# TJUMMG/OCPG

Measured on AMD Instinct MI355X. Metric: clips/sec fwd+bwd (5x384x640, R101), higher is better.
Workload: dtype bf16

## Files before the change

include/ocpg_hip.h:

```cpp
#ifndef OCPG_HIP_H
#define OCPG_HIP_H
#include <stdint.h>

#ifdef __cplusplus
extern "C" {
#endif

int ocpg_msda_fwd_f32(const float* value, const int64_t* shapes, const int64_t* level_start,
                      const float* loc, const float* attn,
                      int N, int S, int M, int D, int L, int Lq, int P,
                      float* out, const int64_t* shapes_host, void* stream);
int ocpg_msda_fwd_f64(const double* value, const int64_t* shapes, const int64_t* level_start,
                      const double* loc, const double* attn,
                      int N, int S, int M, int D, int L, int Lq, int P,
                      double* out, void* stream);

int ocpg_msda_bwd_f32(const float* value, const int64_t* shapes, const int64_t* level_start,
                      const float* loc, const float* attn, const float* grad_out,
                      int N, int S, int M, int D, int L, int Lq, int P,
                      float* grad_value, float* grad_loc, float* grad_attn,
                      const int64_t* shapes_host, void* stream);
int ocpg_msda_bwd_value_f32(const float* loc, const float* attn, const float* grad_out,
                            int N, int S, int M, int D, int L, int Lq, int P,
                            float* grad_value, const int64_t* shapes_host, void* stream);
int ocpg_msda_bwd_locattn_f32(const float* value, const int64_t* shapes, const int64_t* level_start,
                              const float* loc, const float* attn, const float* grad_out,
                              int N, int S, int M, int D, int L, int Lq, int P,
                              float* grad_loc, float* grad_attn, void* stream);
int ocpg_msda_fused_fwd_f32(const float* value, const int64_t* shapes, const int64_t* level_start,
                            const float* qproj, const float* ref,
                            int N, int S, int M, int D, int L, int Lq, int P,
                            float* out, float* loc_out, float* attn_out, void* stream);
int ocpg_msda_fused_bwd_qproj_f32(const float* value, const int64_t* shapes, const int64_t* level_start,
                                  const float* loc, const float* attn, const float* grad_out,
                                  int N, int S, int M, int D, int L, int Lq, int P,
                                  float* grad_qproj, void* stream);
int ocpg_msda_bwd_value_sel_f32(const float* loc, const float* attn, const float* grad_out,
                                int N, int S, int M, int D, int L, int Lq, int P,
                                float* grad_value, const int64_t* shapes_host, int* sel_state, void* stream);
int ocpg_msda_bwd_f64(const double* value, const int64_t* shapes, const int64_t* level_start,
                      const double* loc, const double* attn, const double* grad_out,
                      int N, int S, int M, int D, int L, int Lq, int P,
                      double* grad_value, double* grad_loc, double* grad_attn, void* stream);

int ocpg_msda_sf_fwd_f32(const float* src, const float* wv, const float* bv, const unsigned char* pad,
                         const int64_t* shapes, const int64_t* level_start, const float* loc, const float* attn,
                         int N, int S, int M, int D, int L, int Lq, int P,
                         float* out, float* s, float* beta, void* stream);
int ocpg_msda_sf_bwd_f32(const float* src, const float* wv, const float* bv, const unsigned char* pad,
                         const int64_t* shapes, const int64_t* level_start, const float* loc, const float* attn,
                         const float* grad_out, int N, int S, int M, int D, int L, int Lq, int P,
                         float* grad_src, float* grad_loc, float* grad_attn, void* stream);
int ocpg_msda_sf_bwd_params_f32(const float* grad_out, const float* s, const float* beta, int N, int M, int D, int Lq,
                                float* grad_wv, float* grad_bv, void* stream);

int ocpg_msda_fwd_h16(const void* value, const int64_t* shapes, const int64_t* level_start,
                      const float* loc, const float* attn,
                      int N, int S, int M, int D, int L, int Lq, int P,
                      void* out, const int64_t* shapes_host, int dtype, void* stream);
int ocpg_msda_bwd_h16(const void* value, const int64_t* shapes, const int64_t* level_start,
                      const float* loc, const float* attn, const void* grad_out,
                      int N, int S, int M, int D, int L, int Lq, int P,
                      float* grad_value, float* grad_loc, float* grad_attn,
                      const int64_t* shapes_host, int* sel_state, int dtype, void* stream);
int ocpg_msda_bwd_value_h16(const float* loc, const float* attn, const void* grad_out,
                            int N, int S, int M, int D, int L, int Lq, int P,
                            float* grad_value, const int64_t* shapes_host, int* sel_state, int dtype, void* stream);
int ocpg_msda_bwd_locattn_h16(const void* value, const int64_t* shapes, const int64_t* level_start,
                              const float* loc, const float* attn, const void* grad_out,
                              int N, int S, int M, int D, int L, int Lq, int P,
                              float* grad_loc, float* grad_attn, int dtype, void* stream);
int ocpg_msda_fused_fwd_h16(const void* value, const int64_t* shapes, const int64_t* level_start,
                            const float* qproj, const float* ref,
                            int N, int S, int M, int D, int L, int Lq, int P,
                            void* out, float* loc_out, float* attn_out, int dtype, void* stream);
int ocpg_msda_fused_bwd_qproj_h16(const void* value, const int64_t* shapes, const int64_t* level_start,
                                  const float* loc, const float* attn, const void* grad_out,
                                  int N, int S, int M, int D, int L, int Lq, int P,
                                  float* grad_qproj, int dtype, void* stream);

int ocpg_bn_act_fwd(const void* x, const float* scale, const float* shift, const void* skip, void* y,
                    long long n_outer, int C, long long inner, int relu, int dtype, void* stream);
int ocpg_bn_act_bwd(const void* gy, const void* y, const float* scale, void* gx, void* gskip,
                    long long n_outer, int C, long long inner, int relu, int dtype, void* stream);

int ocpg_gemm_dgrad_bn_tile(long long M, int N, int K);
int ocpg_gemm_dgrad_bn(const void* a, const void* w, const void* c, const void* mask, const float* scale, void* out, void* out_skip,
                       long long M, int N, int K, int dtype, int tile, void* stream);

int ocpg_win_attn_fwd(const void* qkv, const float* biasT, const int* region, float scale, int BW, int NW, int N, int H,
                      int head_dim, void* out, float* lse, int dtype, void* stream);
int ocpg_win_attn_bwd(const void* qkv, const float* bias, const float* biasT, const int* region, float scale, int BW, int NW,
                      int N, int H, int head_dim, const void* out, const void* dout, const float* lse, void* dqkv, float* Dbuf,
                      float* dbiasT, int dtype, void* stream);

int ocpg_win_attn_bwd_mfma(const void* qkv, const float* bias, const float* biasT, const int* region, float scale, int BW, int NW, int N,
                           int H, int head_dim, const void* out, const void* dout, const float* lse, void* dqkv, float* Dbuf, void* dS,
                           int dtype, void* stream);

int ocpg_win_attn_dtable_supported(int N, int head_dim, int dtype, int T);
int ocpg_win_attn_bwd_mfma_dtable(const void* qkv, const float* bias, const float* biasT, const int* region, float scale, int BW, int NW,
                                  int N, int H, int head_dim, const void* out, const void* dout, const float* lse, void* dqkv, float* Dbuf,
                                  const int* tok_code, int code_off, int T, float* partials, float* dtable, int dtype, void* stream);

int ocpg_dynmask_fwd_f32(const float* feats, const float* params, const float* refpix, int BT, int Q, int C, int H, int W,
                         int stride, float* out, float* pre1, void* stream);

int ocpg_dynmask_bwd_pre_f32(const float* dout, const float* pre1, const float* params, int BT, int Q, int C, int H, int W,
                             int stride, float* dpre, float* part, float* w0d, void* stream);
int ocpg_dynmask_bwd_fin_f32(const float* part, const float* params, const float* refpix, const float* dw0, int BT, int Q, int C,
                             int H, int W, float* dparams, float* dref, void* stream);

int ocpg_im2col3x3_nhwc(const void* x, int N, int H, int W, int C, int stride, int dil, void* cols, int dtype, void* stream);
int ocpg_col2im3x3_nhwc(const void* dcols, int N, int H, int W, int C, int stride, int dil, void* dx, int dtype, void* stream);

int ocpg_conv3x3_mfma_fwd(const void* x, const void* w, const float* scale, const float* bias, int relu, int N, int H, int W,
                          int Cin, int Cout, int stride, void* y, void* stream);
int ocpg_conv3x3_mfma_fwd_cols(const void* x, const void* w, const float* scale, const float* bias, int relu, int N, int H, int W, int Cin,
                               int Cout, int stride, void* y, void* cols, void* stream);
int ocpg_conv3x3_mfma_dgrad(const void* dy, const void* wT, int N, int H, int W, int Cin, int Cout, int stride, void* dx,
                            void* stream);
int ocpg_conv3x3_mfma_dgrad_masked(const void* dy, const void* wT, const void* mask_y, const float* scale, int N, int H, int W, int Cin,
                                   int Cout, int stride, void* dx, void* stream);
int ocpg_conv3x3_mfma_dgrad_w(const void* dy, const void* w, const void* mask_y, const float* scale, int N, int H, int W, int Cin, int Cout,
                              int stride, void* dx, void* stream);
int ocpg_conv3x3_mfma_body_splits(long long M, int ncols, int kchannels);
int ocpg_conv3x3_mfma_fwd_bn_splitk(const void* x, const void* w, const float* scale, const float* shift, int relu, int N, int H, int W, int Cin,
                                    int Cout, int stride, int splits, float* part, void* y, void* stream);
int ocpg_conv3x3_mfma_dgrad_w_splitk(const void* dy, const void* w, const void* mask_y, const float* scale, int N, int H, int W, int Cin,
                                     int Cout, int stride, int splits, float* part, void* dx, void* stream);
int ocpg_conv3x3_mfma_wgrad_splits(int N, int H, int W, int Cin, int Cout, int stride);
int ocpg_conv3x3_mfma_wgrad(const void* gz, const void* x, int N, int H, int W, int Cin, int Cout, int stride, void* part, void* stream);
int ocpg_conv3x3_mfma_fwd_cols_h16(const void* x, const void* w, const float* scale, const float* bias, int relu, int N, int H, int W, int Cin,
                                   int Cout, int stride, void* y, void* cols, int dtype, void* stream);
int ocpg_conv3x3_mfma_dgrad_w_h16(const void* dy, const void* w, const void* mask_y, const float* scale, int N, int H, int W, int Cin, int Cout,
                                  int stride, void* dx, int dtype, void* stream);
int ocpg_conv3x3_mfma_wgrad_h16(const void* gz, const void* x, int N, int H, int W, int Cin, int Cout, int stride, void* part, int dtype,
                                void* stream);
int ocpg_conv3x3_mfma_dgrad_w_s2(const void* dy, const void* w, const void* mask_y, const float* scale, int N, int H, int W, int Cin, int Cout,
                                 int stride, void* dx, void* stream);
int ocpg_conv3x3_mfma_dgrad_w_s2_h16(const void* dy, const void* w, const void* mask_y, const float* scale, int N, int H, int W, int Cin, int Cout,
                                     int stride, void* dx, int dtype, void* stream);

int ocpg_conv3x3_mfma_splits(int N, int H, int W, int Cin, int Cout, int stride);
int ocpg_conv3x3_mfma_fwd_splitk(const void* x, const void* w, const float* bias, int N, int H, int W, int Cin, int Cout, int stride,
                                 int splits, float* part, void* y, int out_dt, void* cols, void* stream);
int ocpg_conv3x3_mfma_fwd_splitk_h16(const void* x, const void* w, const float* bias, int N, int H, int W, int Cin, int Cout, int stride,
                                     int splits, float* part, void* y, int out_dt, void* cols, int dtype, void* stream);

int ocpg_gemm(const void* A, const void* B, void* C, const void* bias, int dtype, int out_dtype, int transA, int transB,
              long long M, long long N, long long K, long long lda, long long ldb, long long ldc, long long batch,
              long long strideA, long long strideB, long long strideC, float alpha, float beta, void* stream);
long long ocpg_gemm_plans(void);
long long ocpg_gemm_tuned(long long* changed);
long long ocpg_gemm_tune_rejected(void);
void ocpg_gemm_set_tuning(int on);
long long ocpg_gemm_export_picks(long long* buf, long long cap_pairs);
int ocpg_gemm_import_picks(const long long* buf, long long n_pairs);
int ocpg_gemm_bn_act(const void* A, const void* W, void* D, const float* scale, const float* shift, const void* skip, int relu, int dtype,
                     long long M, long long N, long long K, void* stream);

int ocpg_levelset_fwd_f32(const float* x, const float* feats, const float* box, int Lr, int N, int C, int CF, int h, int w, float* sums,
                          float* coef, float* loss, void* stream);
int ocpg_levelset_bwd_f32(const float* x, const float* feats, const float* box, const float* coef, const float* gloss, int Lr, int N,
                          int C, int CF, int h, int w, float* gx, float* gfeat, void* stream);
int ocpg_proj_fwd_f32(const float* x, const float* tcmax, const float* trmax, const float* tcmean, const float* trmean, int Lr, int B,
                      int T, int H, int W, float* colstat, float* rowstat, float* IU, float* loss, void* stream);
int ocpg_proj_bwd_f32(const float* x, const float* tcmax, const float* trmax, const float* tcmean, const float* trmean,
                      const float* colstat, const float* rowstat, const float* IU, const float* gloss, int Lr, int B, int T, int H, int W,
                      float* Gc, float* Gr, float* gx, void* stream);

int ocpg_matcher_cost_f32(const float* logits, const float* boxes, const float* masks, long long sl, long long sb, long long st,
                          long long sq, const float* gt, const float* tboxes, const float* valid, const long long* labels, int Lr,
                          int B, int T, int Q, int K, int h, int w, float wc, float wb, float wg, float wm, float wd, float* sums,
                          float* cost, int* bad, void* stream);

int ocpg_dropout_add_ln_fwd(const void* x, const float* res, const float* gamma, const float* beta, long long R, int C, float eps, float p,
                            unsigned long long seed, unsigned long long offset, const unsigned long long* rng_base, int x_dtype, float* y,
                            float* mean, float* rstd, void* stream);
int ocpg_dropout_add_ln_bwd(const float* gy, const void* x, const float* res, const float* gamma, const float* mean, const float* rstd,
                            long long R, int C, float p, unsigned long long seed, unsigned long long offset, const unsigned long long* rng_base,
                            int x_dtype, void* gx, float* gres, float* dgb_part, void* stream);
long long ocpg_dropout_add_ln_bwd_slots(long long R);
int ocpg_dropout_add_ln_fwd_ex(const void* x, const float* res, const float* gamma, const float* beta, long long R, int C, float eps, float p,
                               unsigned long long seed, unsigned long long offset, const unsigned long long* rng_base, int x_dtype, float* y,
                               float* mean, float* rstd, const float* addend, float* y_add, void* y_lp, int lp_dtype, void* stream);
int ocpg_dropout_add_ln_bwd_ex(const void* g0, int g0_dtype, const void* g1, int g1_dtype, const void* g2, int g2_dtype, const void* x,
                               const float* res, const float* gamma, const float* mean, const float* rstd, long long R, int C, float p,
                               unsigned long long seed, unsigned long long offset, const unsigned long long* rng_base, int x_dtype, void* gx,
                               float* gres, float* dgb_part, float* gxsum_part, void* stream);
int ocpg_bias_relu_dropout_fwd(const void* a, const void* bias, long long R, int C, float p, unsigned long long seed,
                               unsigned long long offset, const unsigned long long* rng_base, int dtype, void* h, void* stream);
int ocpg_bias_relu_dropout_bwd(const void* gh, const void* h, long long R, int C, float p, int dtype, void* ga, float* dbias_part,
                               void* stream);
long long ocpg_bias_relu_dropout_bwd_slots(long long R, int C, int dtype);

int ocpg_multi_cast(const long long* srcs, const long long* dsts, const long long* numels, const long long* chunk_prefix, int n,
                    long long total_chunks, int src_dtype, int dst_dtype, void* stream);
int ocpg_multi_cast_sum(const long long* srcs, const long long* dsts, const long long* numels, const long long* chunk_prefix,
                        const long long* splits, const long long* strides, int n, long long total_chunks, int src_dtype, int dst_dtype,
                        void* stream);
long long ocpg_colsum_blocks(long long R);
int ocpg_colsum_partials(const void* x, long long R, int C, int dtype, float* part, void* stream);

int ocpg_grad_norm_clip(const long long* grads, const long long* numels, const long long* chunk_prefix, int n, long long total_chunks,
                        float max_norm, float* partials, float* norm_and_coef, void* stream);
int ocpg_adamw_step(const long long* params, const long long* grads, const long long* exp_avg, const long long* exp_avg_sq,
                    const long long* numels, const long long* chunk_prefix, const float* lr, const float* weight_decay, int n,
                    long long total_chunks, const float* norm_and_coef, double beta1, double beta2, double eps, long long step, void* stream);
int ocpg_grad_norm_clip_amp(const long long* grads, const long long* numels, const long long* chunk_prefix, int n, long long total_chunks,
                            float max_norm, float* partials, const float* grad_scale, const float* found_inf, double beta1, double beta2,
                            float* amp_state, void* stream);
int ocpg_adamw_step_amp(const long long* params, const long long* grads, const long long* exp_avg, const long long* exp_avg_sq,
                        const long long* numels, const long long* chunk_prefix, const float* lr, const float* weight_decay, int n,
                        long long total_chunks, const float* amp_state, double beta1, double beta2, double eps, void* stream);

int ocpg_det_loss_fwd_f32(const float* logits, const float* boxes, const long long* src, const float* valid, const long long* labels,
                          const float* tboxes, const float* num_boxes, float alpha, int Lr, int B, int T, int Q, int K, float* loss, int* bad,
                          void* stream);
int ocpg_det_loss_bwd_f32(const float* logits, const float* boxes, const long long* src, const float* valid, const long long* labels,
                          const float* tboxes, const float* num_boxes, const float* gloss, float alpha, int Lr, int B, int T, int Q, int K,
                          float* glogits, float* gboxes, void* stream);

int ocpg_spectral_gate_fwd(const void* X, const float* coef, const float* high, int N, int C, int hw, float* out, void* stream);
int ocpg_spectral_c2p(const void* X, const float* coef, const float* high, int N, int C, int hw, void* pair, int dtype, void* stream);
int ocpg_spectral_p2c(const void* pair, const void* Xs, const float* coef, const float* high, int N, int C, int hw, void* out, float* part,
                      int dtype, void* stream);
int ocpg_spectral_gate_bwd(const float* gout, const void* X, const float* coef, const float* high, int N, int C, int hw, void* dX, float* part,
                           void* stream);

int ocpg_masked_ce_fwd_f32(const float* x, const float* w, const float* t, int Lr, long long per_layer, float* part, void* stream);
int ocpg_masked_ce_bwd_f32(const float* x, const float* w, const float* t, const float* gloss, int Lr, long long per_layer, float* gx,
                           void* stream);

int ocpg_attn_smallk_fwd(const void* q, long long ldq, const void* k, long long ldk, const void* v, long long ldv,
                         const unsigned char* key_pad, float scale, int Lq, int B, int H, int hd, int Lk, float pdrop,
                         unsigned long long seed, unsigned long long offset, const unsigned long long* rng_base, void* out,
                         long long ldo, float* lse, int dtype, void* stream);
int ocpg_attn_smallk_bwd(const void* q, long long ldq, const void* k, long long ldk, const void* v, long long ldv,
                         const unsigned char* key_pad, const void* dout, long long ldo, const float* lse, float scale, int Lq,
                         int B, int H, int hd, int Lk, float pdrop, unsigned long long seed, unsigned long long offset,
                         const unsigned long long* rng_base, void* dq, long long lddq, float* dk, float* dv, int dtype, void* stream);

int ocpg_attn_longk_fwd(const void* q, long long ldq, const void* k, long long ldk, const void* v, long long ldv,
                        const unsigned char* key_pad, float scale, int Lq, int B, int H, int hd, int Lk, float pdrop,
                        unsigned long long seed, unsigned long long offset, const unsigned long long* rng_base, void* out,
                        long long ldo, float* lse, int dtype, void* stream);
int ocpg_attn_longk_bwd(const void* q, long long ldq, const void* k, long long ldk, const void* v, long long ldv,
                        const unsigned char* key_pad, const void* dout, long long ldo, const void* out, long long ldout,
                        const float* lse, float scale, int Lq, int B, int H, int hd, int Lk, float pdrop, unsigned long long seed,
                        unsigned long long offset, const unsigned long long* rng_base, void* dq, long long lddq, float* dk, float* dv,
                        int dtype, void* stream);

int ocpg_lfm_dft_supported(int H, int W);
int ocpg_lfm_dft_split(int L);
int ocpg_lfm_spectrum_fwd(const float* x, const float* coef, const float* high, int N, int H, int W, int C, const void* tw_h, const void* tw_w,
                          float norm, void* tmp, void* pair, int pair_dt, void* stream);
int ocpg_lfm_spectrum_inv(const void* pair, int pair_dt, const float* coef, const float* high, const void* z_saved, float* coef_part, int N, int H,
                          int W, int C, const void* tw_h, const void* tw_w, float norm, void* tmp, const float* residual, float* out, void* stream);
int ocpg_window_means3x3_fwd(const float* x, long long planes, int h, int w, int as_bf16, float* out, void* stream);
int ocpg_window_means3x3_bwd(const float* gm, long long planes, int h, int w, float* dx, void* stream);
int ocpg_window_sums3x3_cl_bands(int h);
int ocpg_window_sums3x3_cl(const float* x, int N, int h, int w, int C, int as_bf16, float* part, void* stream);
int ocpg_window_means3x3_bwd_cl(const float* gm, int N, int h, int w, int C, const float* addend, float* dx, void* stream);

int ocpg_mso_conv3x3(const void* in, int in_dt, int relu_in, const void* w, int w_dt, const float* bias, const float* addend, int NA,
                     const void* mask, int mask_dt, const float* residual, void* out, int out_dt, int NB, int H, int W, int C,
                     int co_total, int compute_dt, void* stream);
int ocpg_mso_wgrad_rows(int NB, int H, int C, int compute_dt);
int ocpg_mso_wgrad(const void* x, int x_dt, int relu_in, const float* g, float* part, float* part_bias, int accumulate, int NB, int H, int W,
                   int C, int co, int rows_per_band, int compute_dt, void* stream);
int ocpg_bilinear_nhwc_fwd(const float* in, int NB, int H, int W, int C, int HO, int WO, float* out, void* stream);
int ocpg_bilinear_nhwc_bwd(const float* gout, int NB, int H, int W, int C, int HO, int WO, float* gin, void* stream);

int ocpg_small_linear_fwd(const void* x, int x_f32, const void* w, const void* b, int R, int Cin, int Cout, int relu, void* y, void* stream);
int ocpg_small_linear_bwd(const void* gy, int gy_f32, const void* x, int x_f32, const void* w, const void* y_relu, int R, int Cin, int Cout,
                          void* gx, void* gw, void* gb, void* stream);
int ocpg_small_linear_fwd_h16(const void* x, int x_f32, const void* w, const void* b, int R, int Cin, int Cout, int relu, void* y, int dtype,
                              void* stream);
int ocpg_small_linear_bwd_h16(const void* gy, int gy_f32, const void* x, int x_f32, const void* w, const void* y_relu, int R, int Cin, int Cout,
                              void* gx, void* gw, void* gb, int dtype, void* stream);
int ocpg_small_linear_f32_fwd(const float* x, const float* w, const float* b, int R, int Cin, int Cout, float* y, void* stream);
int ocpg_small_linear_f32_bwd(const float* gy, const float* x, const float* w, int R, int Cin, int Cout, float* gx, float* gw, float* gb, void* stream);

int ocpg_layernorm_blocks(long long rows);
int ocpg_layernorm_fwd(const void* x, int x_f32, const float* gamma, const float* beta, long long rows, int C, float eps, void* y, int y_f32,
                       float* mean, float* rstd, void* stream);
int ocpg_layernorm_bwd(const void* gy, int gy_f32, const void* x, int x_f32, const float* gamma, const float* mean, const float* rstd,
                       long long rows, int C, void* dx, int dx_f32, float* part_g, float* part_b, void* stream);

long long ocpg_groupnorm_cl_work(long long N, int HW, int C, int G);
int ocpg_groupnorm_cl_fwd(const void* x, int x_dtype, const float* gamma, const float* beta, long long N, int HW, int C, int G, float eps,
                          float* y, float* mean, float* rstd, float* work, void* stream);
int ocpg_groupnorm_cl_bwd(const float* gy, const void* x, int x_dtype, const float* gamma, const float* mean, const float* rstd, long long N,
                          int HW, int C, int G, void* dx, float* part, float* work, void* stream);
int ocpg_groupnorm_cl2cl_fwd(const void* x, int x_dtype, const float* gamma, const float* beta, long long N, int HW, int C, int G, float eps,
                             float* y, float* mean, float* rstd, float* work, void* stream);
int ocpg_groupnorm_cl2cl_bwd(const float* gy, const void* x, int x_dtype, const float* gamma, const float* mean, const float* rstd, long long N,
                             int HW, int C, int G, void* dx, float* part, float* work, void* stream);

int ocpg_gather_rows_bwd(const float* g, const long long* order, const long long* seg, int T, int H, float* out, void* stream);
int ocpg_relpos_bias_fwd(const float* table, const long long* idx, int N, long long ldi, int H, float* bias, float* bias_t, void* stream);
int ocpg_relpos_bias_bwd(const float* g, const long long* order, const long long* seg, int T, int H, int N, int transposed, float* out,
                         void* stream);

int ocpg_gather_rows_pad(const void* x, const long long* idx, long long B, long long S, long long M, long long row_bytes, void* out,
                         void* stream);

int ocpg_graph_replace_memsets(void* hip_graph, int* n_replaced);
int ocpg_graph_stats(void* hip_graph, long long* out9);
int ocpg_graph_memcpy_nodes(void* hip_graph, long long* out, int cap);

int ocpg_text_gate_rows(int Lk);
int ocpg_text_gate_splits(int L);
int ocpg_text_gate_fwd_h16(const float* x, const void* Kp, const void* Vp, const float* c, const float* bo, const unsigned char* key_pad,
                           float scale, int B, int L, int C, int H, int Lk, float* out, int dtype, void* stream);
int ocpg_text_gate_bwd_h16(const float* x, const float* g, const void* Kp, const void* Vp, const float* c, const float* bo,
                           const unsigned char* key_pad, float scale, int B, int L, int C, int H, int Lk, float* dx, float* part, void* ws,
                           int dtype, void* stream);

int ocpg_mask_tail_f32(const float* src, int K, int N, int hs, int ws, int up, int crop_h, int crop_w, int out_h, int out_w, int mode,
                       float thr, float bg, int on_value, void* out, void* stream);

int ocpg_jf_counts_u8(const unsigned char* gt, const unsigned char* res, int T, int H, int W, int G, int R, int radius, int void_label,
                      int all_pairs, int* counts, void* stream);

long long ocpg_sim_heat_workspace(int F, int h, int w, int total);
int ocpg_sim_heat_f32(const float* feat, int F, int h, int w, int C, int n_obj, const int* obj_frame, const int* cand_off_host,
                      const int* cand_off, const int* cand_xy, const int* box, float* heat, int* choice, float* score, void* workspace,
                      void* stream);

int ocpg_refmask_counts_f32(const float* src, int B, int Q, int hs, int ws, int up, const int* geom_host, const int* geom,
                            const unsigned char* gt, const long long* gt_off, int max_out_h, int max_out_w, float thr, int invert,
                            int* counts, void* stream);

const char* ocpg_hip_version(void);

#ifdef __cplusplus
}
#endif
#endif
```

ocpg_amd/_lib.py:

```python
import ctypes
import os

import torch

_HERE = os.path.dirname(os.path.abspath(__file__))
LIB_PATH = os.environ.get("OCPG_HIP_LIB") or os.path.join(_HERE, "lib", "libocpg_hip.so")
_lib = None

_i64p = ctypes.c_void_p
_vp = ctypes.c_void_p
_int = ctypes.c_int

SIGNATURES = {
    "ocpg_msda_fwd_f32": [_vp, _i64p, _i64p, _vp, _vp] + [_int] * 7 + [_vp, _vp, _vp],
    "ocpg_msda_fwd_f64": [_vp, _i64p, _i64p, _vp, _vp] + [_int] * 7 + [_vp, _vp],
    "ocpg_msda_bwd_f32": [_vp, _i64p, _i64p, _vp, _vp, _vp] + [_int] * 7 + [_vp, _vp, _vp, _vp, _vp],
    "ocpg_msda_bwd_value_f32": [_vp, _vp, _vp] + [_int] * 7 + [_vp, _vp, _vp],
    "ocpg_msda_fused_fwd_f32": [_vp, _i64p, _i64p, _vp, _vp] + [_int] * 7 + [_vp, _vp, _vp, _vp],
    "ocpg_msda_fused_bwd_qproj_f32": [_vp, _i64p, _i64p, _vp, _vp, _vp] + [_int] * 7 + [_vp, _vp],
    "ocpg_msda_bwd_value_sel_f32": [_vp, _vp, _vp] + [_int] * 7 + [_vp, _vp, _vp, _vp],
    "ocpg_msda_bwd_locattn_f32": [_vp, _i64p, _i64p, _vp, _vp, _vp] + [_int] * 7 + [_vp, _vp, _vp],
    "ocpg_msda_bwd_f64": [_vp, _i64p, _i64p, _vp, _vp, _vp] + [_int] * 7 + [_vp, _vp, _vp, _vp],
    "ocpg_msda_sf_fwd_f32": [_vp, _vp, _vp, _vp, _i64p, _i64p, _vp, _vp] + [_int] * 7 + [_vp, _vp, _vp, _vp],
    "ocpg_msda_sf_bwd_f32": [_vp, _vp, _vp, _vp, _i64p, _i64p, _vp, _vp, _vp] + [_int] * 7 + [_vp, _vp, _vp, _vp],
    "ocpg_msda_sf_bwd_params_f32": [_vp, _vp, _vp] + [_int] * 4 + [_vp, _vp, _vp],
    "ocpg_msda_fwd_h16": [_vp, _i64p, _i64p, _vp, _vp] + [_int] * 7 + [_vp, _vp, _int, _vp],
    "ocpg_msda_bwd_h16": [_vp, _i64p, _i64p, _vp, _vp, _vp] + [_int] * 7 + [_vp, _vp, _vp, _vp, _vp, _int, _vp],
    "ocpg_msda_bwd_value_h16": [_vp, _vp, _vp] + [_int] * 7 + [_vp, _vp, _vp, _int, _vp],
    "ocpg_msda_bwd_locattn_h16": [_vp, _i64p, _i64p, _vp, _vp, _vp] + [_int] * 7 + [_vp, _vp, _int, _vp],
    "ocpg_msda_fused_fwd_h16": [_vp, _i64p, _i64p, _vp, _vp] + [_int] * 7 + [_vp, _vp, _vp, _int, _vp],
    "ocpg_msda_fused_bwd_qproj_h16": [_vp, _i64p, _i64p, _vp, _vp, _vp] + [_int] * 7 + [_vp, _int, _vp],
    "ocpg_bn_act_fwd": [_vp, _vp, _vp, _vp, _vp, ctypes.c_longlong, _int, ctypes.c_longlong, _int, _int, _vp],
    "ocpg_bn_act_bwd": [_vp, _vp, _vp, _vp, _vp, ctypes.c_longlong, _int, ctypes.c_longlong, _int, _int, _vp],
    "ocpg_gemm_dgrad_bn_tile": [ctypes.c_longlong, _int, _int],
    "ocpg_gemm_dgrad_bn": [_vp] * 7 + [ctypes.c_longlong, _int, _int, _int, _int, _vp],
    "ocpg_dynmask_fwd_f32": [_vp, _vp, _vp] + [_int] * 6 + [_vp, _vp, _vp],
    "ocpg_dynmask_bwd_pre_f32": [_vp, _vp, _vp] + [_int] * 6 + [_vp, _vp, _vp, _vp],
    "ocpg_dynmask_bwd_fin_f32": [_vp, _vp, _vp, _vp] + [_int] * 5 + [_vp, _vp, _vp],
    "ocpg_conv3x3_mfma_fwd": [_vp, _vp, _vp, _vp] + [_int] * 7 + [_vp, _vp],
    "ocpg_conv3x3_mfma_fwd_cols": [_vp, _vp, _vp, _vp] + [_int] * 7 + [_vp, _vp, _vp],
    "ocpg_conv3x3_mfma_dgrad": [_vp, _vp] + [_int] * 6 + [_vp, _vp],
    "ocpg_conv3x3_mfma_dgrad_masked": [_vp, _vp, _vp, _vp] + [_int] * 6 + [_vp, _vp],
    "ocpg_conv3x3_mfma_dgrad_w": [_vp, _vp, _vp, _vp] + [_int] * 6 + [_vp, _vp],
    "ocpg_conv3x3_mfma_splits": [_int] * 6,
    "ocpg_conv3x3_mfma_wgrad_splits": [_int] * 6,
    "ocpg_conv3x3_mfma_body_splits": [ctypes.c_longlong, _int, _int],
    "ocpg_conv3x3_mfma_fwd_bn_splitk": [_vp, _vp, _vp, _vp] + [_int] * 8 + [_vp, _vp, _vp],
    "ocpg_conv3x3_mfma_dgrad_w_splitk": [_vp, _vp, _vp, _vp] + [_int] * 7 + [_vp, _vp, _vp],
    "ocpg_conv3x3_mfma_wgrad": [_vp, _vp] + [_int] * 6 + [_vp, _vp],
    "ocpg_conv3x3_mfma_fwd_cols_h16": [_vp, _vp, _vp, _vp] + [_int] * 7 + [_vp, _vp, _int, _vp],
    "ocpg_conv3x3_mfma_dgrad_w_h16": [_vp, _vp, _vp, _vp] + [_int] * 6 + [_vp, _int, _vp],
    "ocpg_conv3x3_mfma_wgrad_h16": [_vp, _vp] + [_int] * 6 + [_vp, _int, _vp],
    "ocpg_conv3x3_mfma_dgrad_w_s2": [_vp, _vp, _vp, _vp] + [_int] * 6 + [_vp, _vp],
    "ocpg_conv3x3_mfma_dgrad_w_s2_h16": [_vp, _vp, _vp, _vp] + [_int] * 6 + [_vp, _int, _vp],
    "ocpg_conv3x3_mfma_fwd_splitk": [_vp, _vp, _vp] + [_int] * 7 + [_vp, _vp, _int, _vp, _vp],
    "ocpg_conv3x3_mfma_fwd_splitk_h16": [_vp, _vp, _vp] + [_int] * 7 + [_vp, _vp, _int, _vp, _int, _vp],
    "ocpg_gemm": [_vp, _vp, _vp, _vp] + [_int] * 4 + [ctypes.c_longlong] * 10 + [ctypes.c_float, ctypes.c_float, _vp],
    "ocpg_gemm_plans": [],
    "ocpg_gemm_tuned": [_vp],
    "ocpg_gemm_tune_rejected": [],
    "ocpg_gemm_set_tuning": [_int],
    "ocpg_gemm_export_picks": [_vp, ctypes.c_longlong],
    "ocpg_gemm_import_picks": [_vp, ctypes.c_longlong],
    "ocpg_window_means3x3_fwd": [_vp, ctypes.c_longlong, _int, _int, _int, _vp, _vp],
    "ocpg_window_means3x3_bwd": [_vp, ctypes.c_longlong, _int, _int, _vp, _vp],
    "ocpg_window_sums3x3_cl_bands": [_int],
    "ocpg_window_sums3x3_cl": [_vp, _int, _int, _int, _int, _int, _vp, _vp],
    "ocpg_window_means3x3_bwd_cl": [_vp, _int, _int, _int, _int, _vp, _vp, _vp],
    "ocpg_mso_conv3x3": [_vp, _int, _int, _vp, _int, _vp, _vp, _int, _vp, _int, _vp, _vp, _int] + [_int] * 6 + [_vp],
    "ocpg_mso_wgrad_rows": [_int] * 4,
    "ocpg_mso_wgrad": [_vp, _int, _int, _vp, _vp, _vp] + [_int] * 8 + [_vp],
    "ocpg_bilinear_nhwc_fwd": [_vp] + [_int] * 6 + [_vp, _vp],
    "ocpg_bilinear_nhwc_bwd": [_vp] + [_int] * 6 + [_vp, _vp],
    "ocpg_small_linear_fwd": [_vp, _int, _vp, _vp, _int, _int, _int, _int, _vp, _vp],
    "ocpg_small_linear_bwd": [_vp, _int, _vp, _int, _vp, _vp, _int, _int, _int, _vp, _vp, _vp, _vp],
    "ocpg_small_linear_fwd_h16": [_vp, _int, _vp, _vp, _int, _int, _int, _int, _vp, _int, _vp],
    "ocpg_small_linear_bwd_h16": [_vp, _int, _vp, _int, _vp, _vp, _int, _int, _int, _vp, _vp, _vp, _int, _vp],
    "ocpg_small_linear_f32_fwd": [_vp, _vp, _vp, _int, _int, _int, _vp, _vp],
    "ocpg_small_linear_f32_bwd": [_vp, _vp, _vp, _int, _int, _int, _vp, _vp, _vp, _vp],
    "ocpg_layernorm_blocks": [ctypes.c_longlong],
    "ocpg_groupnorm_cl_work": [ctypes.c_longlong, _int, _int, _int],
    "ocpg_groupnorm_cl_fwd": [_vp, _int, _vp, _vp, ctypes.c_longlong, _int, _int, _int, ctypes.c_float, _vp, _vp, _vp, _vp, _vp],
    "ocpg_groupnorm_cl_bwd": [_vp, _vp, _int, _vp, _vp, _vp, ctypes.c_longlong, _int, _int, _int, _vp, _vp, _vp, _vp],
    "ocpg_groupnorm_cl2cl_fwd": [_vp, _int, _vp, _vp, ctypes.c_longlong, _int, _int, _int, ctypes.c_float, _vp, _vp, _vp, _vp, _vp],
    "ocpg_groupnorm_cl2cl_bwd": [_vp, _vp, _int, _vp, _vp, _vp, ctypes.c_longlong, _int, _int, _int, _vp, _vp, _vp, _vp],
    "ocpg_layernorm_fwd": [_vp, _int, _vp, _vp, ctypes.c_longlong, _int, ctypes.c_float, _vp, _int, _vp, _vp, _vp],
    "ocpg_layernorm_bwd": [_vp, _int, _vp, _int, _vp, _vp, _vp, ctypes.c_longlong, _int, _vp, _int, _vp, _vp, _vp],
    "ocpg_gather_rows_bwd": [_vp, _vp, _vp, _int, _int, _vp, _vp],
    "ocpg_relpos_bias_fwd": [_vp, _vp, _int, ctypes.c_longlong, _int, _vp, _vp, _vp],
    "ocpg_relpos_bias_bwd": [_vp, _vp, _vp, _int, _int, _int, _int, _vp, _vp],
    "ocpg_gather_rows_pad": [_vp, _vp] + [ctypes.c_longlong] * 4 + [_vp, _vp],
    "ocpg_graph_replace_memsets": [_vp, _vp],
    "ocpg_graph_stats": [_vp, _vp],
    "ocpg_graph_memcpy_nodes": [_vp, _vp, _int],
    "ocpg_gemm_bn_act": [_vp] * 6 + [_int, _int] + [ctypes.c_longlong] * 3 + [_vp],
    "ocpg_levelset_fwd_f32": [_vp] * 3 + [_int] * 6 + [_vp] * 4,
    "ocpg_levelset_bwd_f32": [_vp] * 5 + [_int] * 6 + [_vp] * 3,
    "ocpg_proj_fwd_f32": [_vp] * 5 + [_int] * 5 + [_vp] * 5,
    "ocpg_proj_bwd_f32": [_vp] * 9 + [_int] * 5 + [_vp] * 4,
    "ocpg_matcher_cost_f32": [_vp] * 3 + [ctypes.c_longlong] * 4 + [_vp] * 4 + [_int] * 7 + [ctypes.c_float] * 5 + [_vp] * 4,
    "ocpg_dropout_add_ln_fwd": [_vp] * 4 + [ctypes.c_longlong, _int, ctypes.c_float, ctypes.c_float, ctypes.c_ulonglong, ctypes.c_ulonglong, _vp, _int]
                               + [_vp] * 4,
    "ocpg_dropout_add_ln_bwd": [_vp] * 6 + [ctypes.c_longlong, _int, ctypes.c_float, ctypes.c_ulonglong, ctypes.c_ulonglong, _vp, _int] + [_vp] * 4,
    "ocpg_dropout_add_ln_bwd_slots": [ctypes.c_longlong],
    "ocpg_dropout_add_ln_fwd_ex": [_vp] * 4 + [ctypes.c_longlong, _int, ctypes.c_float, ctypes.c_float, ctypes.c_ulonglong, ctypes.c_ulonglong, _vp, _int]
                                  + [_vp] * 6 + [_int, _vp],
    "ocpg_dropout_add_ln_bwd_ex": [_vp, _int] * 3 + [_vp] * 5 + [ctypes.c_longlong, _int, ctypes.c_float, ctypes.c_ulonglong, ctypes.c_ulonglong, _vp, _int]
                                  + [_vp] * 5,
    "ocpg_bias_relu_dropout_fwd": [_vp, _vp, ctypes.c_longlong, _int, ctypes.c_float, ctypes.c_ulonglong, ctypes.c_ulonglong, _vp, _int, _vp, _vp],
    "ocpg_bias_relu_dropout_bwd": [_vp, _vp, ctypes.c_longlong, _int, ctypes.c_float, _int, _vp, _vp, _vp],
    "ocpg_bias_relu_dropout_bwd_slots": [ctypes.c_longlong, _int, _int],
    "ocpg_multi_cast": [_vp] * 4 + [_int, ctypes.c_longlong, _int, _int, _vp],
    "ocpg_multi_cast_sum": [_vp] * 6 + [_int, ctypes.c_longlong, _int, _int, _vp],
    "ocpg_colsum_blocks": [ctypes.c_longlong],
    "ocpg_grad_norm_clip": [_vp] * 3 + [_int, ctypes.c_longlong, ctypes.c_float, _vp, _vp, _vp],
    "ocpg_adamw_step": [_vp] * 8 + [_int, ctypes.c_longlong, _vp, ctypes.c_double, ctypes.c_double, ctypes.c_double, ctypes.c_longlong, _vp],
    "ocpg_grad_norm_clip_amp": [_vp] * 3 + [_int, ctypes.c_longlong, ctypes.c_float, _vp, _vp, _vp, ctypes.c_double, ctypes.c_double, _vp, _vp],
    "ocpg_adamw_step_amp": [_vp] * 8 + [_int, ctypes.c_longlong, _vp, ctypes.c_double, ctypes.c_double, ctypes.c_double, _vp],
    "ocpg_lfm_dft_supported": [_int, _int],
    "ocpg_lfm_dft_split": [_int],
    "ocpg_lfm_spectrum_fwd": [_vp, _vp, _vp] + [_int] * 4 + [_vp, _vp, ctypes.c_float, _vp, _vp, _int, _vp],
    "ocpg_lfm_spectrum_inv": [_vp, _int, _vp, _vp, _vp, _vp] + [_int] * 4 + [_vp, _vp, ctypes.c_float, _vp, _vp, _vp, _vp],
    "ocpg_colsum_partials": [_vp, ctypes.c_longlong, _int, _int, _vp, _vp],
    "ocpg_det_loss_fwd_f32": [_vp] * 7 + [ctypes.c_float] + [_int] * 5 + [_vp] * 3,
    "ocpg_det_loss_bwd_f32": [_vp] * 8 + [ctypes.c_float] + [_int] * 5 + [_vp] * 3,
    "ocpg_spectral_gate_fwd": [_vp] * 3 + [_int] * 3 + [_vp, _vp],
    "ocpg_spectral_gate_bwd": [_vp] * 4 + [_int] * 3 + [_vp, _vp, _vp],
    "ocpg_spectral_c2p": [_vp] * 3 + [_int] * 3 + [_vp, _int, _vp],
    "ocpg_spectral_p2c": [_vp] * 4 + [_int] * 3 + [_vp, _vp, _int, _vp],
    "ocpg_masked_ce_fwd_f32": [_vp] * 3 + [_int, ctypes.c_longlong, _vp, _vp],
    "ocpg_masked_ce_bwd_f32": [_vp] * 4 + [_int, ctypes.c_longlong, _vp, _vp],
    "ocpg_im2col3x3_nhwc": [_vp] + [_int] * 6 + [_vp, _int, _vp],
    "ocpg_col2im3x3_nhwc": [_vp] + [_int] * 6 + [_vp, _int, _vp],
    "ocpg_attn_smallk_fwd": [_vp, ctypes.c_longlong, _vp, ctypes.c_longlong, _vp, ctypes.c_longlong, _vp, ctypes.c_float] + [_int] * 5
                            + [ctypes.c_float, ctypes.c_ulonglong, ctypes.c_ulonglong, _vp, _vp, ctypes.c_longlong, _vp, _int, _vp],
    "ocpg_attn_smallk_bwd": [_vp, ctypes.c_longlong, _vp, ctypes.c_longlong, _vp, ctypes.c_longlong, _vp, _vp, ctypes.c_longlong, _vp,
                             ctypes.c_float] + [_int] * 5 + [ctypes.c_float, ctypes.c_ulonglong, ctypes.c_ulonglong, _vp, _vp, ctypes.c_longlong,
                                                             _vp, _vp, _int, _vp],
    "ocpg_attn_longk_fwd": [_vp, ctypes.c_longlong, _vp, ctypes.c_longlong, _vp, ctypes.c_longlong, _vp, ctypes.c_float] + [_int] * 5
                           + [ctypes.c_float, ctypes.c_ulonglong, ctypes.c_ulonglong, _vp, _vp, ctypes.c_longlong, _vp, _int, _vp],
    "ocpg_attn_longk_bwd": [_vp, ctypes.c_longlong, _vp, ctypes.c_longlong, _vp, ctypes.c_longlong, _vp, _vp, ctypes.c_longlong, _vp,
                            ctypes.c_longlong, _vp, ctypes.c_float] + [_int] * 5 + [ctypes.c_float, ctypes.c_ulonglong, ctypes.c_ulonglong, _vp,
                                                                                    _vp, ctypes.c_longlong, _vp, _vp, _int, _vp],
    "ocpg_text_gate_rows": [_int],
    "ocpg_text_gate_splits": [_int],
    "ocpg_text_gate_fwd_h16": [_vp] * 6 + [ctypes.c_float] + [_int] * 5 + [_vp, _int, _vp],
    "ocpg_text_gate_bwd_h16": [_vp] * 7 + [ctypes.c_float] + [_int] * 5 + [_vp, _vp, _vp, _int, _vp],
    "ocpg_mask_tail_f32": [_vp] + [_int] * 10 + [ctypes.c_float, ctypes.c_float, _int, _vp, _vp],
    "ocpg_jf_counts_u8": [_vp, _vp] + [_int] * 8 + [_vp, _vp],
    "ocpg_refmask_counts_f32": [_vp] + [_int] * 5 + [_vp] * 4 + [_int, _int, ctypes.c_float, _int, _vp, _vp],
    "ocpg_sim_heat_workspace": [_int] * 4,
    "ocpg_sim_heat_f32": [_vp] + [_int] * 5 + [_vp] * 10,
    "ocpg_win_attn_fwd": [_vp, _vp, _vp, ctypes.c_float] + [_int] * 5 + [_vp, _vp, _int, _vp],
    "ocpg_win_attn_bwd": [_vp, _vp, _vp, _vp, ctypes.c_float] + [_int] * 5 + [_vp] * 6 + [_int, _vp],
    "ocpg_win_attn_bwd_mfma": [_vp, _vp, _vp, _vp, ctypes.c_float] + [_int] * 5 + [_vp] * 6 + [_int, _vp],
    "ocpg_win_attn_dtable_supported": [_int] * 4,
    "ocpg_win_attn_bwd_mfma_dtable": [_vp, _vp, _vp, _vp, ctypes.c_float] + [_int] * 5 + [_vp] * 6 + [_int, _int, _vp, _vp, _int, _vp],
}


_TIMING = {"on": False, "events": []}
_UNTIMED = ("ocpg_sim_heat_workspace", "ocpg_text_gate_rows", "ocpg_text_gate_splits", "ocpg_win_attn_dtable_supported", "ocpg_conv3x3_mfma_body_splits", "ocpg_gemm_dgrad_bn_tile", "ocpg_conv3x3_mfma_wgrad_splits", "ocpg_window_sums3x3_cl_bands", "ocpg_lfm_dft_supported", "ocpg_lfm_dft_split", "ocpg_conv3x3_mfma_splits", "ocpg_gemm_set_tuning", "ocpg_gemm_export_picks", "ocpg_gemm_import_picks", "ocpg_colsum_blocks", "ocpg_mso_wgrad_rows", "ocpg_gemm_plans", "ocpg_gemm_tuned", "ocpg_gemm_tune_rejected", "ocpg_bias_relu_dropout_bwd_slots", "ocpg_dropout_add_ln_bwd_slots", "ocpg_groupnorm_cl_work")


def enable_kernel_timing(on=True):
    _TIMING["on"] = on
    _TIMING["events"] = []


def collect_kernel_timing(work=None):
    torch.cuda.synchronize()
    out = {}
    for name, args, e0, e1 in _TIMING["events"]:
        d = out.setdefault(name, {"ms": 0.0, "n": 0, "work": 0.0, "modelled": 0})
        d["ms"] += e0.elapsed_time(e1)
        d["n"] += 1
        w = work(name, args) if work is not None else None
        if isinstance(w, tuple):
            d["work_lowp"] = d.get("work_lowp", 0.0) + (w[0] if w[1] else 0.0)
            w = w[0]
        if w is not None:
            d["work"] += w
            d["modelled"] += 1
    _TIMING["events"] = []
    _TIMING["on"] = False
    return out


CENSUS = {"on": False, "calls": {}}
CENSUS_ALSO = {"ocpg_conv3x3_mfma_dgrad_w_s2": "ocpg_conv3x3_mfma_dgrad_w", "ocpg_conv3x3_mfma_dgrad_w_s2_h16": "ocpg_conv3x3_mfma_dgrad_w_h16",
               "ocpg_dropout_add_ln_fwd_ex": "ocpg_dropout_add_ln_fwd", "ocpg_dropout_add_ln_bwd_ex": "ocpg_dropout_add_ln_bwd"}


def census(on=True):
    CENSUS["on"] = on
    if on:
        CENSUS["calls"] = {}
    return CENSUS["calls"]


class _Lib:

    def __init__(self, cdll):
        self._cdll = cdll

    def __getattr__(self, name):
        fn = getattr(self._cdll, name)
        if name not in SIGNATURES or name in _UNTIMED:
            setattr(self, name, fn)
            return fn
        timed = not name.startswith("ocpg_msda_")

        def call(*a):
            if CENSUS["on"]:
                rc = fn(*a)
                if rc == 0:
                    for k in (name, CENSUS_ALSO.get(name)):
                        if k is not None:
                            CENSUS["calls"][k] = CENSUS["calls"].get(k, 0) + 1
                return rc
            if not (timed and _TIMING["on"]):
                return fn(*a)
            e0, e1 = torch.cuda.Event(enable_timing=True), torch.cuda.Event(enable_timing=True)
            e0.record()
            rc = fn(*a)
            e1.record()
            _TIMING["events"].append((name, tuple(getattr(x, "value", x) for x in a), e0, e1))
            return rc
        setattr(self, name, call)
        return call


def lib():
    global _lib
    if _lib is None:
        if not os.path.exists(LIB_PATH):
            raise RuntimeError(
                f"{LIB_PATH} not found: build it with `python -m ocpg_amd.csrc.build` "
                "(hipcc --offload-arch=gfx950). The HIP extension is mandatory; there is no CPU/PyTorch fallback.")
        L = ctypes.CDLL(LIB_PATH)
        for name, argtypes in SIGNATURES.items():
            fn = getattr(L, name)
            fn.argtypes = argtypes
            fn.restype = ctypes.c_int
        L.ocpg_hip_version.restype = ctypes.c_char_p
        L.ocpg_gemm_plans.restype = ctypes.c_longlong
        L.ocpg_gemm_tuned.restype = ctypes.c_longlong
        L.ocpg_gemm_tune_rejected.restype = ctypes.c_longlong
        L.ocpg_gemm_export_picks.restype = ctypes.c_longlong
        L.ocpg_gemm_set_tuning.restype = None
        L.ocpg_bias_relu_dropout_bwd_slots.restype = ctypes.c_longlong
        L.ocpg_dropout_add_ln_bwd_slots.restype = ctypes.c_longlong
        L.ocpg_groupnorm_cl_work.restype = ctypes.c_longlong
        L.ocpg_colsum_blocks.restype = ctypes.c_longlong
        L.ocpg_sim_heat_workspace.restype = ctypes.c_longlong
        _lib = _Lib(L)
    return _lib


def check(status, what):
    if status != 0:
        if status <= -1000:
            raise RuntimeError(f"{what}: invalid argument #{-status - 1000}")
        raise RuntimeError(f"{what}: HIP error {-status}")


def stream_ptr():
    return ctypes.c_void_p(torch.cuda.current_stream().cuda_stream)


def require_gpu(name, t):
    if not t.is_cuda:
        raise RuntimeError(f"{name} must be a GPU tensor: Not implemented on the CPU")
    if not t.is_contiguous():
        raise RuntimeError(f"{name} tensor has to be contiguous")
```

ocpg_amd/csrc/levelset.hip:

```cpp
#include <hip/hip_runtime.h>
#include <stdint.h>

#include "../../include/ocpg_hip.h"
#include "fill.h"

namespace {

constexpr int CMAX = 16;
constexpr float EPS_W = 0.00001f;
constexpr int PPT = 4;

__device__ __forceinline__ float sigmoidf_(float x) { return 1.f / (1.f + __expf(-x)); }
__device__ __forceinline__ float sgnf_(float v) { return (v > 0.f) - (v < 0.f); }

__device__ __forceinline__ float wave_sum(float v) {
#pragma unroll
  for (int o = 32; o > 0; o >>= 1) v += __shfl_down(v, o, 64);
  return v;
}

__global__ __launch_bounds__(256) void levelset_sums(const float* __restrict__ x, const float* __restrict__ feats,
                                                     const float* __restrict__ box, int N, int C, int CF, int h, int w,
                                                     float* __restrict__ sums) {
  const int hw = h * w;
  const int n = blockIdx.y, l = blockIdx.z;
  const int NS = 7 + 2 * C;
  float acc[7 + 2 * CMAX];
#pragma unroll
  for (int i = 0; i < 7 + 2 * CMAX; ++i) acc[i] = 0.f;
  const float* xl = x + ((long long)l * N + n) * hw;
  const float* bx = box + (long long)n * hw;
#pragma unroll 1
  for (int it = 0; it < PPT; ++it) {
    const int px = blockIdx.x * (256 * PPT) + it * 256 + threadIdx.x;
    if (px >= hw) break;
    const float b = bx[px];
    const float p = sigmoidf_(xl[px]);
    const float fg = p * b, bg = (1.f - p) * b;
    const int yy = px / w, xx = px % w;
    if (yy + 1 < h) {
      const float pd = sigmoidf_(xl[px + w]), bd = bx[px + w];
      acc[4] += fabsf(pd * bd - fg);
      acc[5] += fabsf((1.f - pd) * bd - bg);
    }
    if (xx + 1 < w) {
      const float pr = sigmoidf_(xl[px + 1]), br = bx[px + 1];
      acc[4] += fabsf(pr * br - fg);
      acc[5] += fabsf((1.f - pr) * br - bg);
    }
    acc[6] += b;
    if (b != 0.f) {
      const float* f = feats + (long long)n * CF * hw + px;
      float t2 = 0.f;
#pragma unroll
      for (int c = 0; c < CMAX; ++c) {
        if (c < C) {
          const float t = f[(long long)c * hw] * b;
          t2 += t * t;
          acc[7 + c] += fg * t;
          acc[7 + CMAX + c] += bg * t;
        }
      }
      acc[0] += fg; acc[1] += bg; acc[2] += fg * t2; acc[3] += bg * t2;
    }
  }
  __shared__ float red[4][7 + 2 * CMAX];
  const int wave = threadIdx.x >> 6, lane = threadIdx.x & 63;
#pragma unroll
  for (int i = 0; i < 7 + 2 * CMAX; ++i) {
    const bool used = i < 7 || (i < 7 + CMAX ? i - 7 < C : i - 7 - CMAX < C);
    if (used) {
      const float v = wave_sum(acc[i]);
      if (lane == 0) red[wave][i] = v;
    }
  }
  __syncthreads();
  if (threadIdx.x < 7 + 2 * CMAX) {
    const int i = threadIdx.x;
    const bool used = i < 7 || (i < 7 + CMAX ? i - 7 < C : i - 7 - CMAX < C);
    if (used) {
      const float v = red[0][i] + red[1][i] + red[2][i] + red[3][i];
      const int slot = i < 7 ? i : (i < 7 + CMAX ? 7 + (i - 7) : 7 + C + (i - 7 - CMAX));
      sums[(((long long)l * N + n) * gridDim.x + blockIdx.x) * NS + slot] = v;
    }
  }
}

__global__ __launch_bounds__(64) void levelset_final(const float* __restrict__ part, int nblk, int N, int C, float* __restrict__ coef,
                                                     float* __restrict__ loss) {
  __shared__ float s[7 + 2 * CMAX];
  const int n = blockIdx.x, l = blockIdx.y;
  const int NS = 7 + 2 * C, NC = 8 + 2 * C;
  const float* p = part + ((long long)l * N + n) * nblk * NS;
  for (int slot = 0; slot < NS; ++slot) {
    float v = 0.f;
    for (int b = threadIdx.x; b < nblk; b += 64) v += p[(long long)b * NS + slot];
    v = wave_sum(v);
    if (threadIdx.x == 0) s[slot] = v;
  }
  __syncthreads();
  if (threadIdx.x != 0) return;
  float* k = coef + ((long long)l * N + n) * NC;
  const float pixels = fmaxf(s[6], 1.f);
  float e_tot = 0.f;
#pragma unroll
  for (int side = 0; side < 2; ++side) {
    const float W = s[side], A = s[2 + side];
    const float D = fmaxf(W, EPS_W);
    const float r = W / D, delta = W > EPS_W ? 1.f : 0.f;
    float cs = 0.f, cc = 0.f;
    for (int c = 0; c < C; ++c) {
      const float S = s[7 + side * C + c];
      const float cv = S / D;
      k[8 + side * C + c] = cv;
      cs += cv * S;
      cc += cv * cv;
    }
    e_tot += A - 2.f * cs + cc * W;
    k[2 * side] = 4.f - 2.f * r;
    k[2 * side + 1] = (1.f + 2.f * delta - 2.f * r * delta) * cc;
    k[4 + side] = 2.f - r;
  }
  k[6] = 1.f / ((float)C * pixels);
  k[7] = 0.00001f / pixels;
  atomicAdd(loss + l, (e_tot / (float)C / pixels + 0.00001f * (s[4] + s[5]) / pixels) / (float)N);
}

__global__ __launch_bounds__(256) void levelset_bwd(const float* __restrict__ x, const float* __restrict__ feats,
                                                    const float* __restrict__ box, const float* __restrict__ coef,
                                                    const float* __restrict__ gloss, int Lr, int N, int C, int CF, int h, int w,
                                                    float* __restrict__ gx, float* __restrict__ gfeat) {
  const int hw = h * w;
  const int n = blockIdx.y;
  const int px = blockIdx.x * 256 + threadIdx.x;
  if (px >= hw) return;
  const int NC = 8 + 2 * C;
  const float* bx = box + (long long)n * hw;
  const float b = bx[px];
  const int yy = px / w, xx = px % w;
  float t[CMAX], gt[CMAX];
  float t2 = 0.f;
  const float* f = feats + (long long)n * CF * hw + px;
#pragma unroll
  for (int c = 0; c < CMAX; ++c) {
    t[c] = (c < C && b != 0.f) ? f[(long long)c * hw] * b : 0.f;
    t2 += t[c] * t[c];
    gt[c] = 0.f;
  }
  const bool up = yy > 0, down = yy + 1 < h, left = xx > 0, right = xx + 1 < w;
  const float b_u = up ? bx[px - w] : 0.f, b_d = down ? bx[px + w] : 0.f, b_l = left ? bx[px - 1] : 0.f, b_r = right ? bx[px + 1] : 0.f;
  for (int l = 0; l < Lr; ++l) {
    const float* xl = x + ((long long)l * N + n) * hw;
    float g = 0.f;
    if (b != 0.f) {
      const float* k = coef + ((long long)l * N + n) * NC;
      const float G = gloss[l] / (float)N;
      const float p = sigmoidf_(xl[px]);
      const float fg = p * b, bg = (1.f - p) * b;
      float dot_f = 0.f, dot_b = 0.f;
#pragma unroll
      for (int c = 0; c < CMAX; ++c) {
        if (c < C) {
          dot_f += k[8 + c] * t[c];
          dot_b += k[8 + C + c] * t[c];
        }
      }
      const float de_f = t2 - k[0] * dot_f + k[1], de_b = t2 - k[2] * dot_b + k[3];
      float dl_f = 0.f, dl_b = 0.f;
      if (up)    { const float q = sigmoidf_(xl[px - w]); dl_f += sgnf_(fg - q * b_u); dl_b += sgnf_(bg - (1.f - q) * b_u); }
      if (down)  { const float q = sigmoidf_(xl[px + w]); dl_f -= sgnf_(q * b_d - fg); dl_b -= sgnf_((1.f - q) * b_d - bg); }
      if (left)  { const float q = sigmoidf_(xl[px - 1]); dl_f += sgnf_(fg - q * b_l); dl_b += sgnf_(bg - (1.f - q) * b_l); }
      if (right) { const float q = sigmoidf_(xl[px + 1]); dl_f -= sgnf_(q * b_r - fg); dl_b -= sgnf_((1.f - q) * b_r - bg); }
      const float gfg = G * (k[6] * de_f + k[7] * dl_f), gbg = G * (k[6] * de_b + k[7] * dl_b);
      g = (gfg - gbg) * p * (1.f - p) * b;
      const float sf = 2.f * G * k[6] * fg, sb = 2.f * G * k[6] * bg;
#pragma unroll
      for (int c = 0; c < CMAX; ++c)
        if (c < C) gt[c] += sf * (t[c] - k[4] * k[8 + c]) + sb * (t[c] - k[5] * k[8 + C + c]);
    }
    gx[((long long)l * N + n) * hw + px] = g;
  }
  if (gfeat) {
    float* gf = gfeat + (long long)n * CF * hw + px;
    for (int c = 0; c < CF; ++c) gf[(long long)c * hw] = c < C ? gt[c < CMAX ? c : 0] * b : 0.f;
  }
}

}

extern "C" {

int ocpg_levelset_fwd_f32(const float* x, const float* feats, const float* box, int Lr, int N, int C, int CF, int h, int w, float* sums,
                          float* coef, float* loss, void* stream) {
  if (Lr <= 0 || N <= 0 || C <= 0 || C > CMAX || CF < C || h <= 0 || w <= 0) return -1006;
  if (N > 65535 || Lr > 65535) return -1007;
  if (!x) return -1001;
  if (!feats) return -1002;
  if (!box) return -1003;
  if (!sums || !coef || !loss) return -1010;
  hipStream_t st = (hipStream_t)stream;
  const int hw = h * w;
  const int nblk = (hw + 256 * PPT - 1) / (256 * PPT);
  hipError_t e = ocpg_fill::zero_async(loss, sizeof(float) * (size_t)Lr, st);
  if (e != hipSuccess) return -(int)e;
  levelset_sums<<<dim3(nblk, N, Lr), 256, 0, st>>>(x, feats, box, N, C, CF, h, w, sums);
  levelset_final<<<dim3(N, Lr), 64, 0, st>>>(sums, nblk, N, C, coef, loss);
  e = hipGetLastError();
  return e == hipSuccess ? 0 : -(int)e;
}

int ocpg_levelset_bwd_f32(const float* x, const float* feats, const float* box, const float* coef, const float* gloss, int Lr, int N,
                          int C, int CF, int h, int w, float* gx, float* gfeat, void* stream) {
  if (Lr <= 0 || N <= 0 || C <= 0 || C > CMAX || CF < C || h <= 0 || w <= 0) return -1006;
  if (N > 65535) return -1007;
  if (!x) return -1001;
  if (!feats) return -1002;
  if (!box) return -1003;
  if (!coef) return -1004;
  if (!gloss) return -1005;
  if (!gx) return -1010;
  const int hw = h * w;
  levelset_bwd<<<dim3((hw + 255) / 256, N), 256, 0, (hipStream_t)stream>>>(x, feats, box, coef, gloss, Lr, N, C, CF, h, w, gx, gfeat);
  const hipError_t e = hipGetLastError();
  return e == hipSuccess ? 0 : -(int)e;
}

}
```

ocpg_amd/models/criterion.py:

```python
import torch
import torch.nn.functional as F
from torch import nn

from ..util import box_ops
from ..util.misc import get_world_size, is_dist_avail_and_initialized, nested_tensor_from_tensor_list
from .matcher import _assert_well_formed, _pairwise_giou_1
from .ops.functions import mask_loss_func
from .segmentation import generate_box_region_mask

HIP_MASK_LOSSES = True
HIP_DET_LOSSES = True


def _pad_stack(targets, key):
    return nested_tensor_from_tensor_list([t[key] for t in targets], size_divisibility=32, split=False).decompose()[0]


def _sub(x, k):
    return x[..., k // 2::k, k // 2::k]


def _dice(x, t):
    inter = (x * t).sum(-1)
    union = (x ** 2.0).sum(-1) + (t ** 2.0).sum(-1) + 1e-5
    return 1.0 - (2 * inter / union)


class SetCriterion(nn.Module):
    def __init__(self, args, num_classes, matcher, weight_dict, eos_coef, losses, focal_alpha=0.25):
        super().__init__()
        self.args = args
        self.num_classes = num_classes
        self.matcher = matcher
        self.weight_dict = weight_dict
        self.eos_coef = eos_coef
        self.losses = losses
        empty_weight = torch.ones(self.num_classes + 1)
        empty_weight[-1] = self.eos_coef
        self.register_buffer("empty_weight", empty_weight)
        self.focal_alpha = focal_alpha
        self.mask_out_stride = 1
        self.mask_out_stride_low = 2
        self.iter = 0
        self._warmup_iters = 100000
        self.iter_device = None

    def _labels_stacked(self, logits, src, targets, num_boxes):
        lr, b, nf, nq, k = logits.shape
        valid = torch.stack([t["valid"] for t in targets]).to(logits.device) > 0
        hit = (torch.arange(nq, device=logits.device).view(1, 1, 1, nq) == src[:, :, None, None]) & valid[None, :, :, None]
        if self.num_classes == 1:
            onehot = hit[..., None].to(logits.dtype)
        else:
            labels = torch.stack([t["labels"] for t in targets]).to(logits.device)
            onehot = (F.one_hot(labels, k)[None, :, :, None, :].bool() & hit[..., None]).to(logits.dtype)
        x, t = logits.reshape(lr, b, nf * nq, k), onehot.reshape(lr, b, nf * nq, k)
        p = x.sigmoid()
        ce = F.binary_cross_entropy_with_logits(x, t, reduction="none")
        p_t = p * t + (1 - p) * (1 - t)
        loss = ce * ((1 - p_t) ** 2)
        if self.focal_alpha >= 0:
            loss = (self.focal_alpha * t + (1 - self.focal_alpha) * (1 - t)) * loss
        return loss.mean(2).sum((1, 2)) / num_boxes * (nf * nq)

    def _boxes_stacked(self, boxes, src, targets, num_boxes):
        lr, b, nf, nq, _ = boxes.shape
        idx = src[:, :, None, None, None].expand(lr, b, nf, 1, 4)
        sel = torch.gather(boxes, 3, idx)[:, :, :, 0]
        tgt = torch.stack([t["boxes"] for t in targets]).to(sel.dtype)[None]
        l1 = (sel - tgt).abs().sum((1, 2, 3)) / num_boxes
        sx, tx = box_ops.box_cxcywh_to_xyxy(sel), box_ops.box_cxcywh_to_xyxy(tgt)
        _assert_well_formed(sx, "predictions")
        _assert_well_formed(tx, "targets")
        giou = (1 - _pairwise_giou_1(sx, tx)).sum((1, 2)) / num_boxes
        return l1, giou

    def _masks_stacked(self, pm, pml, src_lst, targets, num_boxes, warm):
        with torch.autocast(device_type=pm.device.type, enabled=False):
            return self._masks_stacked_fp32(pm.float(), pml.float(), src_lst.float(), targets, num_boxes, warm)

    def _masks_stacked_fp32(self, pm, pml, src_lst, targets, num_boxes, warm):
        lr = pm.shape[0]
        gt = _pad_stack(targets, "masks").to(pml)
        heat = _pad_stack(targets, "weights").to(pml)
        weak = _pad_stack(targets, "weak_masks").to(pml)
        s, sl = self.mask_out_stride, self.mask_out_stride_low
        im_h, im_w = gt.shape[-2:]
        b, nf = weak.shape[:2]
        gt_full = _sub(gt, s)
        assert gt_full.size(2) * s == im_h and gt_full.size(3) * s == im_w
        sizes = torch.stack([t["size"] for t in targets]).repeat_interleave(nf, dim=0)
        boxes = box_ops.box_cxcywh_to_xyxy(torch.cat([t["boxes"] for t in targets], dim=0))
        region = generate_box_region_mask(boxes, (im_h, im_w), sizes).view(b, nf, im_h, im_w)
        region_low, region = _sub(region, sl), _sub(region, s)
        weak_full, weak_low = _sub(weak, s) * region, _sub(weak, sl) * region_low

        def heat_weight(h, reg):
            w = (h.clamp(min=0.3, max=0.7) - 0.5).abs()
            lo, hi = w.min(), w.max()
            w = (w - lo) / (hi - lo + 1e-5)
            return torch.where(reg == 0, torch.ones_like(w), w)

        def masked_ce(x, w, m):
            return F.binary_cross_entropy_with_logits(x.sigmoid() * w, (m * w).expand_as(x), reduction="none").mean((1, 2, 3, 4))

        def proj(x, reg, m):
            p = x.sigmoid()
            ly = _dice(p.amax(3).flatten(2), reg.amax(2).flatten(1)[None])
            lx = _dice(p.amax(4).flatten(2), reg.amax(3).flatten(1)[None])
            my = _dice(p.mean(3).flatten(2), m.mean(2).flatten(1)[None])
            mx = _dice(p.mean(4).flatten(2), m.mean(3).flatten(1)[None])
            return (ly + lx).mean(1) + 0.1 * (my + mx).mean(1)

        def levelset(x, feats, box):
            p = x.sigmoid()
            fg, bg = p * box, (1.0 - p) * box
            pixels = box.sum((1, 2)).clamp(min=1)
            tgt = feats * box[:, None]
            c_in = torch.einsum("lnhw,nchw->lnc", fg, tgt) / fg.sum((2, 3)).clamp(min=0.00001)[..., None]
            c_out = torch.einsum("lnhw,nchw->lnc", bg, tgt) / bg.sum((2, 3)).clamp(min=0.00001)[..., None]
            t2 = (tgt ** 2).sum(1)
            def energy(wgt, c):
                return ((wgt * t2).sum((2, 3)) - 2 * (c * torch.einsum("lnhw,nchw->lnc", wgt, tgt)).sum(-1)
                        + (c ** 2).sum(-1) * wgt.sum((2, 3)))
            region_e = (energy(fg, c_in) + energy(bg, c_out)) / tgt.shape[1]
            def length(v):
                return (v[..., 1:, :] - v[..., :-1, :]).abs().sum((2, 3)) + (v[..., :, 1:] - v[..., :, :-1]).abs().sum((2, 3))
            return (region_e / pixels + 0.00001 * (length(fg) + length(bg)) / pixels).mean(1)

        w_full, w_low = heat_weight(_sub(heat, s), region), heat_weight(_sub(heat, sl), region_low)
        if pm.is_cuda and HIP_MASK_LOSSES and pm[0].numel() % 4 == 0 and pml[0].numel() % 4 == 0:
            loss_mask, loss_mask_low = mask_loss_func.masked_ce(pm, w_full, weak_full), mask_loss_func.masked_ce(pml, w_low, weak_low)
        else:
            loss_mask, loss_mask_low = masked_ce(pm, w_full, weak_full), masked_ce(pml, w_low, weak_low)
        lst_hw = src_lst.shape[-2:]
        scaled = F.interpolate(pm.flatten(0, 1), lst_hw, mode="bilinear", align_corners=True).view(lr, b * nf, *lst_hw)
        region_scaled = F.interpolate(region, lst_hw, mode="nearest").flatten(0, 1)
        feats = src_lst.flatten(0, 1)[:, :-1]
        if pm.is_cuda and HIP_MASK_LOSSES and feats.shape[1] <= 16:
            full_feats = src_lst.flatten(0, 1)
            ls = mask_loss_func.levelset_loss(scaled, full_feats, region_scaled, feats.shape[1])
            ls_low = mask_loss_func.levelset_loss(pml.flatten(1, 2), full_feats, region_scaled, feats.shape[1])
            pj, pj_low = mask_loss_func.proj_loss(pm, region, weak_full), mask_loss_func.proj_loss(pml, region_low, weak_low)
        else:
            ls = levelset(scaled, feats, region_scaled)
            ls_low = levelset(pml.flatten(1, 2), feats, region_scaled)
            pj, pj_low = proj(pm, region, weak_full), proj(pml, region_low, weak_low)
        out = {
            "loss_proj": pj, "loss_mask": (1 - warm) * loss_mask, "loss_lst": warm * ls,
            "loss_proj_low": pj_low, "loss_mask_low": (1 - warm) * loss_mask_low, "loss_lst_low": warm * ls_low,
        }
        return out, (pm[0].sigmoid(), gt_full, weak_full)

    @staticmethod
    def _src_index(indices):
        return torch.cat([src for (src, _) in indices])

    def _get_src_permutation_idx(self, indices):
        batch_idx = torch.cat([torch.full_like(src, i) for i, (src, _) in enumerate(indices)])
        return batch_idx, self._src_index(indices)

    def loss_labels(self, outputs, targets, indices, num_boxes, log=True):
        v = self._labels_stacked(outputs["pred_logits"][None], self._src_index(indices)[None], targets, num_boxes)
        return {"loss_ce": v[0]}, None, None, None

    def loss_boxes(self, outputs, targets, indices, num_boxes):
        l1, giou = self._boxes_stacked(outputs["pred_boxes"][None], self._src_index(indices)[None], targets, num_boxes)
        return {"loss_bbox": l1[0], "loss_giou": giou[0]}, None, None, None

    def loss_masks(self, outputs, targets, indices, num_boxes):
        d, maps = self._masks_stacked(outputs["pred_masks"][None], outputs["pred_masks_low"][None], outputs["ls_features"],
                                      targets, num_boxes, self._warm(1).to(outputs["pred_masks"].device))
        return {k: v[0] for k, v in d.items()}, maps[0], maps[1], maps[2]

    def get_loss(self, loss, outputs, targets, indices, num_boxes, **kwargs):
        table = {"labels": self.loss_labels, "boxes": self.loss_boxes, "masks": self.loss_masks}
        assert loss in table, f"do you really want to compute {loss} loss?"
        return table[loss](outputs, targets, indices, num_boxes, **kwargs)

    def _warm(self, n):
        if self.iter_device is not None:
            k = torch.arange(1, n + 1, device=self.iter_device.device, dtype=torch.float32)
            return torch.clamp((self.iter_device + k) / float(self._warmup_iters), max=1.0)
        w = [min(float(self.iter + i) / float(self._warmup_iters), 1.0) for i in range(1, n + 1)]
        self.iter += n
        return torch.tensor(w)

    @staticmethod
    def global_num_boxes(targets, device):
        num_boxes = torch.stack([t["valid"] for t in targets]).sum().to(device=device, dtype=torch.float).reshape(1)
        if is_dist_avail_and_initialized():
            torch.distributed.all_reduce(num_boxes)
        return torch.clamp(num_boxes / get_world_size(), min=1)[0]

    def forward(self, outputs, targets):
        aux = outputs.get("aux_outputs", [])
        aux_indices = outputs["aux_matcher_index"] if aux else []
        assert len(aux_indices) == len(aux), "Aux index len not match."
        layers = [outputs] + list(aux)
        src = torch.stack([self._src_index(i) for i in [outputs["main_matcher_index"]] + list(aux_indices)])
        num_boxes = outputs.get("num_boxes")
        if num_boxes is None:
            num_boxes = self.global_num_boxes(targets, outputs["pred_logits"].device)
        pre = outputs.get("_stacked")

        def stacked(key):
            if pre is not None and key in pre:
                return pre[key]
            return torch.stack([l[key] for l in layers])

        losses, maps = {}, (None, None, None)
        per_layer = {}
        if HIP_DET_LOSSES and "labels" in self.losses and "boxes" in self.losses and src.is_cuda:
            from .matcher import _BOX_ERRORS
            dev = src.device
            flag = _BOX_ERRORS.get(dev)
            if flag is None and not torch.cuda.is_current_stream_capturing():
                flag = _BOX_ERRORS[dev] = torch.zeros((), dtype=torch.int32, device=dev)
            valid = torch.stack([t["valid"] for t in targets]).to(dev)
            labels = None if self.num_classes == 1 else torch.stack([t["labels"] for t in targets]).to(dev)
            tboxes = torch.stack([t["boxes"] for t in targets]).to(dev)
            det = mask_loss_func.det_losses(stacked("pred_logits"), stacked("pred_boxes"), src, valid, labels, tboxes, num_boxes,
                                            self.focal_alpha, flag)
            per_layer["loss_ce"], per_layer["loss_bbox"], per_layer["loss_giou"] = det.unbind(0)
        else:
            if "labels" in self.losses:
                per_layer["loss_ce"] = self._labels_stacked(stacked("pred_logits"), src, targets, num_boxes)
            if "boxes" in self.losses:
                per_layer["loss_bbox"], per_layer["loss_giou"] = self._boxes_stacked(stacked("pred_boxes"), src, targets, num_boxes)
        if "masks" in self.losses:
            warm = self._warm(len(layers)).to(outputs["pred_masks_low"].device)
            d, maps = self._masks_stacked(stacked("pred_masks"), stacked("pred_masks_low"), outputs["ls_features"], targets, num_boxes, warm)
            per_layer.update(d)
        order = [k for k in ("loss_ce", "loss_bbox", "loss_giou", "loss_proj", "loss_mask", "loss_lst", "loss_proj_low", "loss_mask_low",
                             "loss_lst_low") if k in per_layer]
        table = torch.stack([per_layer[k] for k in order])
        names = [[k if i == 0 else f"{k}_{i - 1}" for i in range(len(layers))] for k in order]
        for i in range(len(layers)):
            for j, row in enumerate(names):
                losses[row[i]] = table[j, i]
        self._last = (losses, table, names)
        return (losses,) + maps

    def weighted_sum(self, loss_dict):
        last = getattr(self, "_last", None)
        if last is None or last[0] is not loss_dict:
            return sum(loss_dict[k] * self.weight_dict[k] for k in loss_dict if k in self.weight_dict)
        _, table, names = last
        self._last = None
        key = (tuple(map(tuple, names)), str(table.device))
        cache = self.__dict__.setdefault("_weight_tables", {})
        w = cache.get(key)
        if w is None:
            w = cache[key] = torch.tensor([[float(self.weight_dict.get(n, 0.0)) for n in row] for row in names], dtype=torch.float32,
                                          device=table.device)
        return (table.float() * w).sum()
```

ocpg_amd/models/matcher.py:

```python
import torch
import torch.nn.functional as F
from torch import nn

from ..util.box_ops import box_cxcywh_to_xyxy
from ..util.misc import nested_tensor_from_tensor_list


def _pairwise_giou_1(boxes, tgt):
    ax0, ay0, ax1, ay1 = boxes.unbind(-1)
    bx0, by0, bx1, by1 = tgt.unbind(-1)
    area_a = (ax1 - ax0) * (ay1 - ay0)
    area_b = (bx1 - bx0) * (by1 - by0)
    inter = (torch.min(ax1, bx1) - torch.max(ax0, bx0)).clamp(min=0) * (torch.min(ay1, by1) - torch.max(ay0, by0)).clamp(min=0)
    union = area_a + area_b - inter
    iou = (inter + 1e-6) / (union + 1e-6)
    hull = (torch.max(ax1, bx1) - torch.min(ax0, bx0)).clamp(min=0) * (torch.max(ay1, by1) - torch.min(ay0, by0)).clamp(min=0)
    return iou - ((hull - union) + 1e-6) / (hull + 1e-6)


HIP_MATCHER = True
_BOX_ERRORS = {}


def _assert_well_formed(xyxy, what):
    ok = (xyxy[..., 2:] >= xyxy[..., :2]).all()
    if xyxy.is_cuda:
        flag = _BOX_ERRORS.get(xyxy.device)
        if flag is None:
            if torch.cuda.is_current_stream_capturing():
                return
            flag = _BOX_ERRORS[xyxy.device] = torch.zeros((), dtype=torch.int32, device=xyxy.device)
        flag += (~ok).to(torch.int32)
    else:
        assert ok, f"error boxes: {what}"


def raise_if_malformed_boxes():
    for dev, flag in _BOX_ERRORS.items():
        n = int(flag.item())
        if n:
            flag.zero_()
            raise AssertionError(f"error boxes: {n} malformed (x1 < x0 or y1 < y0, or NaN) box set(s) seen on {dev}")


class HungarianMatcher(nn.Module):
    def __init__(self, cost_class: float = 1, cost_bbox: float = 1, cost_giou: float = 1, cost_mask: float = 1,
                 cost_dice: float = 1, cost_boundary: float = 1, num_classes: int = 1):
        super().__init__()
        self.cost_class, self.cost_bbox, self.cost_giou = cost_class, cost_bbox, cost_giou
        self.cost_mask, self.cost_dice, self.cost_boundary = cost_mask, cost_dice, cost_boundary
        self.num_classes = num_classes
        assert cost_class != 0 or cost_bbox != 0 or cost_giou != 0 or cost_mask != 0 or cost_dice != 0, "all costs cant be 0"
        self.mask_out_stride = 2

    @torch.no_grad()
    def cost_matrix_stacked(self, logits, boxes, masks, targets):
        with torch.autocast(device_type=masks.device.type, enabled=False):
            logits, boxes, masks = logits.float(), boxes.float(), masks.float()
            lr, bs, nf, nq, h, w = masks.shape
            gt, _ = nested_tensor_from_tensor_list([t["masks"] for t in targets], size_divisibility=32, split=False).decompose()
            gt = gt.to(masks)
            s = self.mask_out_stride
            im_h, im_w = gt.shape[-2:]
            gt = gt[:, :, s // 2::s, s // 2::s]
            assert gt.size(2) * s == im_h and gt.size(3) * s == im_w

            valid = torch.stack([t["valid"] for t in targets]).to(logits.dtype)
            if masks.is_cuda and HIP_MATCHER:
                return self._cost_matrix_hip(logits, boxes, masks, gt, valid, targets)
            prob = logits.sigmoid()
            alpha, gamma = 0.25, 2.0
            neg = (1 - alpha) * (prob ** gamma) * (-(1 - prob + 1e-8).log())
            pos = alpha * ((1 - prob) ** gamma) * (-(prob + 1e-8).log())
            if self.num_classes == 1:
                cls = (pos - neg)[..., 0]
            else:
                ids = torch.stack([t["labels"] for t in targets])
                cls = torch.gather(pos - neg, 4, ids[None, :, :, None, None].expand(lr, -1, -1, nq, 1))[..., 0]
            cost_class = (cls * valid[None, :, :, None]).sum(2) / valid.sum(1)[None, :, None]

            tb = torch.stack([t["boxes"] for t in targets]).to(boxes.dtype)
            cost_bbox = (boxes - tb[None, :, :, None, :]).abs().sum(-1).mean(2)
            pb, tbx = box_cxcywh_to_xyxy(boxes), box_cxcywh_to_xyxy(tb)
            _assert_well_formed(pb, "predictions")
            _assert_well_formed(tbx, "targets")
            cost_giou = -_pairwise_giou_1(pb, tbx[None, :, :, None, :]).mean(2)

            x = masks.transpose(2, 3).flatten(3)
            g = gt.flatten(1)[None, :, None, :]
            p = x.sigmoid()
            ce = F.binary_cross_entropy_with_logits(x, g.expand_as(x), reduction="none")
            p_t = p * g + (1 - p) * (1 - g)
            focal = (alpha * g + (1 - alpha) * (1 - g)) * ce * ((1 - p_t) ** gamma)
            cost_mask = focal.mean(3)
            cost_dice = -((2 * (p * g).sum(3) + 1) / (p.sum(-1) + g.sum(-1) + 1))
            return (self.cost_class * cost_class + self.cost_bbox * cost_bbox + self.cost_giou * cost_giou
                    + self.cost_mask * cost_mask + self.cost_dice * cost_dice)

    def _cost_matrix_hip(self, logits, boxes, masks, gt, valid, targets):
        from .._lib import check, lib
        lr, bs, nf, nq, h, w = masks.shape
        if masks.stride(-1) != 1 or masks.stride(-2) != w:
            masks = masks.contiguous()
        logits, boxes, gt = logits.contiguous(), boxes.contiguous(), gt.contiguous()
        tb = torch.stack([t["boxes"] for t in targets]).to(boxes.dtype).contiguous()
        labels = None if self.num_classes == 1 else torch.stack([t["labels"] for t in targets]).to(torch.int64).contiguous()
        flag = _BOX_ERRORS.get(masks.device)
        if flag is None and not torch.cuda.is_current_stream_capturing():
            flag = _BOX_ERRORS[masks.device] = torch.zeros((), dtype=torch.int32, device=masks.device)
        cost = torch.empty((lr, bs, nq), dtype=torch.float32, device=masks.device)
        sums = torch.empty((lr, bs, nq, 4), dtype=torch.float32, device=masks.device)
        sl, sb, st, sq = masks.stride()[:4]
        check(lib().ocpg_matcher_cost_f32(logits.data_ptr(), boxes.data_ptr(), masks.data_ptr(), sl, sb, st, sq, gt.data_ptr(), tb.data_ptr(),
                                          valid.contiguous().data_ptr(), None if labels is None else labels.data_ptr(), lr, bs, nf, nq,
                                          logits.shape[-1], h, w, float(self.cost_class), float(self.cost_bbox), float(self.cost_giou),
                                          float(self.cost_mask), float(self.cost_dice), sums.data_ptr(), cost.data_ptr(),
                                          None if flag is None else flag.data_ptr(), torch.cuda.current_stream().cuda_stream),
              "ocpg_matcher_cost_f32")
        return cost

    @torch.no_grad()
    def cost_matrix(self, outputs, targets):
        return self.cost_matrix_stacked(outputs["pred_logits"][None], outputs["pred_boxes"][None], outputs["pred_masks"][None], targets)[0]

    @torch.no_grad()
    def match_stacked(self, logits, boxes, masks, targets):
        return self.cost_matrix_stacked(logits, boxes, masks, targets).argmin(dim=2)

    @staticmethod
    def as_indices(src):
        zero = torch.zeros(1, dtype=torch.int64, device=src.device)
        return [(src[i:i + 1], zero) for i in range(src.shape[0])]

    @torch.no_grad()
    def forward(self, outputs, targets):
        return self.as_indices(self.cost_matrix(outputs, targets).argmin(dim=1))


def build_matcher(args):
    if args.binary:
        num_classes = 1
    else:
        num_classes = {"ytvos": 65, "davis": 78, "a2d": 1, "jhmdb": 1}.get(args.dataset_file, 91)
    return HungarianMatcher(cost_class=args.set_cost_class, cost_bbox=args.set_cost_bbox, cost_giou=args.set_cost_giou,
                            cost_mask=args.set_cost_mask, cost_dice=args.set_cost_dice,
                            cost_boundary=args.set_cost_boundary, num_classes=num_classes)
```

ocpg_amd/models/ocpg.py:

```python
import copy
import math
import os
from types import SimpleNamespace

import torch
import torch.nn.functional as F
from torch import nn

from ..util.misc import NestedTensor, inverse_sigmoid, nested_tensor_from_videos_list, resize_mask
from . import amp_cache
from .backbone import build_backbone
from .criterion import SetCriterion
from .decoder import MSO
from .deformable_transformer import build_deforamble_transformer
from .matcher import build_matcher
from .modules import LFMResizeAdaptive
from .ops.functions.dynmask_func import dynamic_mask
from .ops.functions.groupnorm_func import GroupNorm
from .position_encoding import PositionEmbeddingSine1D
from .postprocessors import build_postprocessors
from .resample import bicubic_resize, bilinear_resize, nearest_upsample

MATMUL_BILINEAR = True
CL_FUSE = os.environ.get("OCPG_CL_FUSE", "1") != "0"
GATE_BF = os.environ.get("OCPG_GATE_BF", "0") != "0"
LS_FEAT_N16 = os.environ.get("OCPG_LS_FEAT_N16", "1") != "0"
from .segmentation import VisionLanguageFusionModule
from .text_encoder.text_encoder import FeatureResizer, PrecomputedText, TextEncoder


def _get_clones(module, n):
    return nn.ModuleList([copy.deepcopy(module) for _ in range(n)])


class MLP(nn.Module):

    def __init__(self, input_dim, hidden_dim, output_dim, num_layers):
        super().__init__()
        self.num_layers = num_layers
        dims = [input_dim] + [hidden_dim] * (num_layers - 1) + [output_dim]
        self.layers = nn.ModuleList(amp_cache.Linear(a, b) for a, b in zip(dims[:-1], dims[1:]))

    def forward(self, x):
        for i, layer in enumerate(self.layers):
            if i < self.num_layers - 1:
                x = amp_cache.linear_relu(x, amp_cache.lookup(layer.weight), None if layer.bias is None else amp_cache.lookup(layer.bias))
            else:
                x = layer(x)
        return x


def compute_locations(h, w, device, stride=1):
    xs = torch.arange(0, w * stride, step=stride, dtype=torch.float32, device=device) + stride // 2
    ys = torch.arange(0, h * stride, step=stride, dtype=torch.float32, device=device) + stride // 2
    gy, gx = torch.meshgrid(ys, xs, indexing="ij")
    return torch.stack((gx.reshape(-1), gy.reshape(-1)), dim=1)


def parse_dynamic_params(params, channels, weight_nums, bias_nums):
    assert params.dim() == 2 and len(weight_nums) == len(bias_nums)
    assert params.size(1) == sum(weight_nums) + sum(bias_nums)
    n, nl = params.size(0), len(weight_nums)
    parts = list(torch.split_with_sizes(params, weight_nums + bias_nums, dim=1))
    weights = [parts[l].reshape(n * channels, -1, 1, 1) for l in range(nl)]
    biases = [parts[nl + l].reshape(n * channels) for l in range(nl)]
    return weights, biases


def _get_src_permutation_idx(indices):
    batch_idx = torch.cat([torch.full_like(src, i) for i, (src, _) in enumerate(indices)])
    src_idx = torch.cat([src for (src, _) in indices])
    return batch_idx, src_idx


class OCPG(nn.Module):
    def __init__(self, args, backbone, transformer, num_classes, num_queries, num_feature_levels, num_frames, mask_dim,
                 dim_feedforward, controller_layers, dynamic_mask_channels, aux_loss=False, with_box_refine=False,
                 two_stage=False, freeze_text_encoder=False, freeze_video_encoder=False, rel_coord=True, matcher=None):
        super().__init__()
        assert two_stage is False, "args.two_stage must be false!"
        self.args = args
        self.matcher = matcher
        self.num_frames = num_frames
        self.num_feature_levels = num_feature_levels
        self.training = not args.eval
        self.num_queries = num_queries
        self.transformer = transformer
        hidden_dim = transformer.d_model
        self.hidden_dim = hidden_dim
        self.aux_loss = aux_loss
        self.with_box_refine = with_box_refine
        self.num_classes = num_classes
        self.class_embed = amp_cache.Linear(hidden_dim, num_classes)
        self.bbox_embed = MLP(hidden_dim, hidden_dim, 4, 3)
        self.ls_feat_viz = amp_cache.Conv2d(hidden_dim, 8, 3, 1, 1)
        self.ls_text_proj = amp_cache.Linear(hidden_dim, 8)
        self.mask_dim = mask_dim
        self.controller_layers = controller_layers
        self.dynamic_mask_channels = dynamic_mask_channels
        self.backbone = backbone
        if freeze_video_encoder:
            for p in self.backbone.parameters():
                p.requires_grad_(False)

        self.text_encoder = TextEncoder(args)
        self.text_pos = PositionEmbeddingSine1D(hidden_dim, normalize=True)
        self.text_proj = FeatureResizer(self.text_encoder.feat_dim, hidden_dim, dropout=0.1)
        self.sentence_proj = FeatureResizer(self.text_encoder.feat_dim, hidden_dim, dropout=0.1)
        self.fusion_module = VisionLanguageFusionModule(d_model=hidden_dim, nhead=8)

        self.query_embed = nn.Embedding(num_queries, hidden_dim)
        if num_feature_levels <= 1:
            raise NotImplementedError
        chans = backbone.num_channels[-3:]
        proj, fft, fft_post = [], [], []
        for cin in chans:
            proj.append(nn.Sequential(amp_cache.Conv2d(cin, hidden_dim, kernel_size=1), GroupNorm(32, hidden_dim)))
            amp_cache.mark_single_use(proj[-1][0])
        cin = chans[-1]
        for _ in range(num_feature_levels - len(chans)):
            proj.append(nn.Sequential(amp_cache.Conv2d(cin, hidden_dim, kernel_size=3, stride=2, padding=1), GroupNorm(32, hidden_dim)))
            cin = hidden_dim
        for _ in range(len(proj)):
            fft.append(LFMResizeAdaptive(hidden_dim, 7))
            fft_post.append(LFMResizeAdaptive(hidden_dim, 7))
        self.input_proj = nn.ModuleList(proj)
        self.input_fft = nn.ModuleList(fft)
        self.input_fft_post = nn.ModuleList(fft_post)

        self.mask_refine = MSO(mask_dim=dynamic_mask_channels, img_dim=backbone.num_channels[:2], out_dim=dynamic_mask_channels)
        self.rel_coord = rel_coord
        self.init_aux_head()
        self.build_controller()
        self.transformer.decoder.compute_samples = False

    def init_aux_head(self):
        prior = 0.01
        self.class_embed.bias.data = torch.ones(self.num_classes) * (-math.log((1 - prior) / prior))
        nn.init.zeros_(self.bbox_embed.layers[-1].weight)
        nn.init.zeros_(self.bbox_embed.layers[-1].bias)
        for proj in self.input_proj:
            nn.init.xavier_uniform_(proj[0].weight, gain=1)
            nn.init.zeros_(proj[0].bias)
        nn.init.xavier_uniform_(self.ls_feat_viz.weight, gain=1)
        nn.init.zeros_(self.ls_feat_viz.bias)
        n_pred = self.transformer.decoder.num_layers
        if self.with_box_refine:
            self.class_embed = _get_clones(self.class_embed, n_pred)
            self.bbox_embed = _get_clones(self.bbox_embed, n_pred)
            nn.init.constant_(self.bbox_embed[0].layers[-1].bias.data[2:], -2.0)
            self.transformer.decoder.bbox_embed = self.bbox_embed
        else:
            nn.init.constant_(self.bbox_embed.layers[-1].bias.data[2:], -2.0)
            self.class_embed = nn.ModuleList([self.class_embed for _ in range(n_pred)])
            self.bbox_embed = nn.ModuleList([self.bbox_embed for _ in range(n_pred)])
            self.transformer.decoder.bbox_embed = None

    def build_controller(self):
        self.in_channels = self.mask_dim
        self.mask_out_stride = 4
        self.mask_feat_stride = 8
        ch = self.dynamic_mask_channels
        self.weight_nums, self.bias_nums = [], []
        for l in range(self.controller_layers):
            cin = (self.in_channels + (2 if self.rel_coord else 0)) if l == 0 else ch
            self.weight_nums.append(cin * ch)
            self.bias_nums.append(ch)
        self.num_gen_params = sum(self.weight_nums) + sum(self.bias_nums)
        self.controller = MLP(self.hidden_dim, self.hidden_dim, self.num_gen_params, 3)
        for layer in self.controller.layers:
            nn.init.zeros_(layer.bias)
            nn.init.xavier_uniform_(layer.weight)

    def forward_text(self, captions, device):
        if isinstance(captions, PrecomputedText) or isinstance(captions[0], str):
            feats, sentence, pad = self.text_encoder(captions, device)
            return NestedTensor(self.text_proj(feats), pad), self.sentence_proj(sentence)
        raise ValueError("Please mask sure the caption is a list of string")

    def _gate_token_major(self, src, b, t, text_words, text_pad, text_pos):
        n, c, h, w = src.shape
        vis = src.view(b, t, c, h, w).permute(1, 3, 4, 0, 2)
        vis = self.fusion_module(visual=vis, text=text_words, text_key_padding_mask=text_pad, text_pos=text_pos, visual_pos=None)
        if CL_FUSE and vis.is_cuda:
            return vis.view(t, h, w, b, c).permute(3, 0, 1, 2, 4).reshape(b * t, h, w, c).permute(0, 3, 1, 2)
        return vis.view(t, h, w, b, c).permute(3, 0, 4, 1, 2).reshape(b * t, c, h, w)

    def _fuse_level(self, l, src, b, t, text_words, text_pad, text_pos, high_filter, shared=None):
        n, c, h, w = src.shape
        src, high_filter = self.input_fft[l](src, high_filter)
        if CL_FUSE and (GATE_BF or self.fusion_module.fused_gate_enabled()) and src.is_cuda and src.permute(0, 2, 3, 1).is_contiguous():
            tokens = src.permute(0, 2, 3, 1).reshape(b, t * h * w, c)
            out = None
            if self.fusion_module.fused_gate_serves(tokens, text_words):
                def token_major(tok):
                    return self._gate_token_major(tok.view(b * t, h, w, c).permute(0, 3, 1, 2), b, t, text_words, text_pad,
                                                  text_pos).permute(0, 2, 3, 1).reshape(b, t * h * w, c)
                out = self.fusion_module.forward_tokens(tokens, text_words, text_pad, text_pos, unfused=None if GATE_BF else token_major,
                                                        shared=shared)
            elif GATE_BF:
                out = self.fusion_module.forward_batch_first(tokens, text_words, text_pad, text_pos)
            if out is not None:
                return self.input_fft_post[l](out.view(b * t, h, w, c).permute(0, 3, 1, 2), high_filter)
        return self.input_fft_post[l](self._gate_token_major(src, b, t, text_words, text_pad, text_pos), high_filter)

    def forward(self, samples, captions, targets):
        with amp_cache.scope(self):
            return self._forward(samples, captions, targets)

    def forward_selected(self, samples, captions, targets):
        if self.training:
            raise RuntimeError("forward_selected is an inference path: call model.eval() first")
        if self.args.dataset_file in ("a2d", "jhmdb") or "refcoco" in self.args.dataset_file:
            raise RuntimeError(f"forward_selected serves the best-query (YTVOS / DAVIS) eval branch only, not {self.args.dataset_file}")
        with amp_cache.scope(self):
            return self._forward(samples, captions, targets, selected=True)

    def _forward(self, samples, captions, targets, selected=False):
        s = self._trunk(samples, captions, targets)
        return self._best_query_masks(s, targets) if selected else self._all_masks(s, targets)

    def _trunk(self, samples, captions, targets):
        if not isinstance(samples, NestedTensor):
            samples = nested_tensor_from_videos_list(samples, 1 if self.training else 16)
        features, visual_pos = self.backbone(samples)
        b = len(targets)
        t = visual_pos[0].shape[0] // b
        dev = visual_pos[0].device

        if "valid_indices" in targets[0]:
            vi = torch.tensor([i * t + tg["valid_indices"] for i, tg in enumerate(targets)]).to(dev)
            for f in features:
                f.tensors, f.mask = f.tensors.index_select(0, vi), f.mask.index_select(0, vi)
            visual_pos = [p.index_select(0, vi) for p in visual_pos]
            samples.mask, samples.tensors = samples.mask.index_select(0, vi), samples.tensors.index_select(0, vi)
            t = 1

        text_features, text_sentence = self.forward_text(captions, device=dev)
        text_pos = self.text_pos(text_features).permute(2, 0, 1)
        text_words, text_pad = text_features.decompose()
        text_words = text_words.permute(1, 0, 2)

        srcs, masks, poses = [], [], []
        high_filter = None
        shared = {}
        n_scales = 3
        for l, (feat, pos_l) in enumerate(zip(features[-n_scales:], visual_pos[-n_scales:])):
            src, mask = feat.decompose()
            assert mask is not None
            src, high_filter = self._fuse_level(l, self.input_proj[l](src), b, t, text_words, text_pad, text_pos, high_filter, shared)
            srcs.append(src), masks.append(mask), poses.append(pos_l)
        for l in range(len(srcs), self.num_feature_levels):
            src = self.input_proj[l](features[-1].tensors if l == n_scales else srcs[-1])
            mask = resize_mask(samples.mask, src.shape[-2:])
            pos_l = self.backbone[1](NestedTensor(src, mask)).to(src.dtype)
            src, high_filter = self._fuse_level(l, src, b, t, text_words, text_pad, text_pos, high_filter, shared)
            srcs.append(src), masks.append(mask), poses.append(pos_l)

        text_embed = text_sentence[:, None, None, :].expand(-1, t, self.num_queries, -1)
        hs, memory, init_reference, inter_references, box_deltas, _, inter_samples = \
            self.transformer(srcs, text_embed, masks, poses, self.query_embed.weight)
        nl = hs.shape[0]

        out = {}
        classes, coords = [], []
        hs_l = hs.unbind(0)
        refs_l = (init_reference,) + tuple(inter_references.unbind(0)[:-1])
        for lvl in range(nl):
            ref = inverse_sigmoid(refs_l[lvl])
            delta = box_deltas[lvl] if box_deltas is not None else self.bbox_embed[lvl](hs_l[lvl])
            if ref.shape[-1] == 4:
                delta = delta + ref
            else:
                assert ref.shape[-1] == 2
                delta = delta + F.pad(ref, (0, 2))
            classes.append(self.class_embed[lvl](hs_l[lvl]))
            coords.append(delta.sigmoid())
        outputs_class = torch.stack(classes).unflatten(1, (b, t))
        outputs_coord = torch.stack(coords).unflatten(1, (b, t))
        out["pred_logits"], out["pred_boxes"] = outputs_class[-1], outputs_coord[-1]

        tar = memory[0].shape[-2:]
        memory_fusion = sum(bicubic_resize(x.float(), tar) for x in memory)
        mask_features = memory_fusion.unflatten(0, (b, t))
        nq = self.num_queries
        params = self.controller(hs.transpose(0, 1)).reshape(b, t * nl * nq, -1)
        refs = inter_references[..., :2].transpose(0, 1).reshape(b, t * nl * nq, 2)
        return SimpleNamespace(out=out, hs=hs, features=features, samples=samples, b=b, t=t, nl=nl, nq=nq, dev=dev, tar=tar,
                               inter_references=inter_references, outputs_class=outputs_class, outputs_coord=outputs_coord,
                               memory_fusion=memory_fusion, mask_features=mask_features, params=params, refs=refs,
                               text_sentence=text_sentence)

    def _best_query_masks(self, s, targets):
        out, b, t, nl, nq = dict(s.out), s.b, s.t, s.nl, s.nq
        scores = out["pred_logits"].sigmoid().mean(1).max(-1)[0]
        best = scores.argmax(-1)
        bi = torch.arange(b, device=s.dev)
        out["pred_logits"] = out["pred_logits"][bi, :, best][:, :, None]
        out["pred_boxes"] = out["pred_boxes"][bi, :, best][:, :, None]
        out["reference_points"] = s.inter_references[-2].unflatten(0, (b, t))[bi, :, best][:, :, None, :2]
        p_best = s.params.view(b, t, nl, nq, -1)[:, :, -1][bi, :, best]
        r_best = s.refs.view(b, t, nl, nq, 2)[:, :, -1][bi, :, best]
        m = self.dynamic_mask_with_coords(s.mask_features, p_best, r_best, targets)
        pm = self.mask_refine(m.flatten(0, 1), s.features[:2])
        out["pred_masks_low"] = pm.squeeze(1).unflatten(0, (b, t))
        out["mask_up"] = 4
        return out

    def _all_masks(self, s, targets):
        out, hs, features, samples, b, t, nl, nq, dev, tar = dict(s.out), s.hs, s.features, s.samples, s.b, s.t, s.nl, s.nq, s.dev, s.tar
        inter_references, outputs_class, outputs_coord = s.inter_references, s.outputs_class, s.outputs_coord
        memory_fusion, mask_features, params, refs, text_sentence = s.memory_fusion, s.mask_features, s.params, s.refs, s.text_sentence
        m_all = self.dynamic_mask_with_coords(mask_features, params, refs, targets)
        sh_all = F.pixel_shuffle(m_all.flatten(0, 1), 4).squeeze(1).view(b, t, nl, nq, 4 * tar[0], 4 * tar[1])
        m_all = m_all.view(b, t, nl, nq, 16, tar[0], tar[1])
        seg_masks = [m_all[:, :, l] for l in range(nl)]
        seg_masks_shuffled = [sh_all[:, :, l] for l in range(nl)]

        if self.training:
            shuffled = sh_all.permute(2, 0, 1, 3, 4, 5)
            with torch.no_grad():
                if self.aux_loss:
                    src_all = self.matcher.match_stacked(outputs_class, outputs_coord, shuffled, targets)
                else:
                    src_all = self.matcher.match_stacked(outputs_class[-1:], outputs_coord[-1:], shuffled[-1:], targets)
                out["pred_masks"] = seg_masks_shuffled[-1]
                out["main_matcher_index"] = self.matcher.as_indices(src_all[-1])
                if self.aux_loss:
                    out["aux_outputs"] = self._set_aux_loss(outputs_class, outputs_coord, seg_masks_shuffled)
                    out["aux_matcher_index"] = [self.matcher.as_indices(src_all[i]) for i in range(nl - 1)]
            if self.aux_loss:
                lsf = self._ls_feat(memory_fusion)
                ls_feat = (bilinear_resize(lsf, (4 * lsf.shape[-2], 4 * lsf.shape[-1]), True) if lsf.is_cuda and MATMUL_BILINEAR
                           else F.interpolate(lsf, scale_factor=4, mode="bilinear", align_corners=True))
                ls_feat = ls_feat.unflatten(0, (b, t))
                txt = self.ls_text_proj(text_sentence)[:, None, :, None, None]
                sim = (ls_feat * txt).sum(dim=2) / ((F.normalize(ls_feat, dim=2) * F.normalize(txt, dim=2)).sum(dim=2) + 1e-5)
                img = (bilinear_resize(samples.tensors, tuple(ls_feat.shape[-2:]), True) if lsf.is_cuda and MATMUL_BILINEAR
                       else F.interpolate(samples.tensors, ls_feat.shape[-2:], mode="bilinear", align_corners=True)).unflatten(0, (b, t))
                ls_features = torch.cat([img, ls_feat, sim.unsqueeze(2)], dim=2)

                seg = m_all.permute(2, 0, 1, 3, 4, 5, 6)
                gi = src_all[:, :, None, None, None, None, None].expand(nl, b, t, 1, 16, tar[0], tar[1])
                picked = torch.gather(seg, 3, gi).squeeze(3).flatten(1, 2)
                refined = self.mask_refine.forward_multi(list(picked.unbind(0)), features[:2], stacked=True)
                refined = nearest_upsample(refined, 4).squeeze(1)
                refined = refined.view(nl, b, t, *refined.shape[-2:])
                gl = src_all[:, :, None, None, None, None].expand(nl, b, t, 1, 4 * tar[0], 4 * tar[1])
                low = torch.gather(shuffled, 3, gl).squeeze(3)
                out["pred_masks"] = refined[-1]
                out["ls_features"] = ls_features
                out["frames"] = img
                out["pred_masks_low"] = low[-1]
                out["aux_outputs"] = self._set_aux_loss_comprehensive(outputs_class, outputs_coord, refined, low, ls_features, img)
                def main_first(x):
                    return torch.roll(x, 1, 0)
                out["_stacked"] = {"pred_logits": main_first(outputs_class), "pred_boxes": main_first(outputs_coord),
                                   "pred_masks": main_first(refined), "pred_masks_low": main_first(low)}
        elif self.args.dataset_file not in ("a2d", "jhmdb") and "refcoco" not in self.args.dataset_file:
            m = seg_masks[-1].view(b, t, self.num_queries, 16, tar[0], tar[1])
            scores = out["pred_logits"].sigmoid().mean(1).max(-1)[0]
            best = scores.argmax(-1)
            bi = torch.arange(b, device=dev)
            out["pred_logits"] = out["pred_logits"][bi, :, best][:, :, None]
            out["pred_boxes"] = out["pred_boxes"][bi, :, best][:, :, None]
            out["reference_points"] = inter_references[-2].unflatten(0, (b, t))[bi, :, best][:, :, None, :2]
            pm = self.mask_refine(m[bi, :, best].flatten(0, 1), features[:2])
            pm = F.interpolate(pm, scale_factor=4).squeeze(1).unflatten(0, (b, t))
            out["pred_masks"] = pm.unsqueeze(2)
        else:
            m = seg_masks[-1].view(b, t, self.num_queries, 16, tar[0], tar[1])
            per_q = []
            for qi in range(self.num_queries):
                pm = self.mask_refine(m[:, :, qi].flatten(0, 1), features[:2])
                per_q.append(F.interpolate(pm, scale_factor=4).squeeze(1).unflatten(0, (b, t)))
            out["pred_masks"] = torch.stack(per_q, dim=2)
        return out

    @torch.jit.unused
    def _ls_feat(self, x):
        conv = self.ls_feat_viz
        if not (LS_FEAT_N16 and x.is_cuda and x.shape[0] <= 65535 and x.dtype in (torch.float32, torch.bfloat16, torch.float16)):
            return conv(x)
        from .decoder import _bias32, _nhwc, _tap_major
        from .ops.functions.mso_func import compute_code, conv3x3_n16
        cdt = compute_code(x.device.type)
        y = conv3x3_n16(_nhwc(x), _tap_major(amp_cache.lookup(conv.weight), cdt), _bias32(conv.bias), cdt=cdt)
        y = y.permute(0, 3, 1, 2)
        return y if cdt == 0 else y.to(torch.get_autocast_dtype(x.device.type))

    def _set_aux_loss(self, outputs_class, outputs_coord, outputs_seg_masks):
        return [{"pred_logits": a, "pred_boxes": b_, "pred_masks": c}
                for a, b_, c in zip(outputs_class[:-1], outputs_coord[:-1], outputs_seg_masks[:-1])]

    @torch.jit.unused
    def _set_aux_loss_comprehensive(self, outputs_class, outputs_coord, seg_masks, seg_masks_low, ls_features, img_ori):
        return [{"pred_logits": a, "pred_boxes": b_, "pred_masks": c, "pred_masks_low": d, "ls_features": ls_features, "frames": img_ori}
                for a, b_, c, d in zip(outputs_class[:-1], outputs_coord[:-1], seg_masks[:-1], seg_masks_low[:-1])]

    def dynamic_mask_with_coords(self, mask_features, mask_head_params, reference_points, targets):
        with torch.autocast(device_type=mask_features.device.type, enabled=False):
            feats = mask_features.float()
            b, t, c, h, w = feats.shape
            nq = reference_points.shape[1] // t
            ch = self.dynamic_mask_channels
            if feats.is_cuda and self.rel_coord and self.controller_layers == 2 and ch == 16:
                sizes = torch.stack([tg["size"] for tg in targets]).to(feats.device, torch.float32)
                refpix = reference_points.float() * torch.stack([sizes[:, 1], sizes[:, 0]], -1)[:, None, :]
                out = dynamic_mask(feats.reshape(b * t, c, h, w), mask_head_params.float().reshape(b * t * nq, -1),
                                   refpix.reshape(b * t * nq, 2), self.mask_feat_stride)
                return out.view(b, t * nq, ch, h, w)
            params = mask_head_params.float().reshape(b, t, nq, -1)
            parts = torch.split_with_sizes(params, self.weight_nums + self.bias_nums, dim=-1)
            n_layers = len(self.weight_nums)
            weights, biases = parts[:n_layers], parts[n_layers:]
            cin0 = c + (2 if self.rel_coord else 0)
            w0 = weights[0].reshape(b, t, nq * ch, cin0)
            x = torch.matmul(w0[..., :c].reshape(b * t, nq * ch, c), feats.reshape(b * t, c, h * w))
            x = x.view(b, t, nq, ch, h, w)
            if self.rel_coord:
                sizes = torch.stack([tg["size"] for tg in targets]).to(feats.device, torch.float32)
                ref = reference_points.float().reshape(b, t, nq, 2) * torch.stack([sizes[:, 1], sizes[:, 0]], -1)[:, None, None, :]
                s = self.mask_feat_stride
                xs = torch.arange(0, w * s, step=s, dtype=torch.float32, device=feats.device) + s // 2
                ys = torch.arange(0, h * s, step=s, dtype=torch.float32, device=feats.device) + s // 2
                wx = w0[..., c].reshape(b, t, nq, ch)
                wy = w0[..., c + 1].reshape(b, t, nq, ch)
                relx = ref[..., 0, None] - xs
                rely = ref[..., 1, None] - ys
                x = x + wx[..., None, None] * relx[:, :, :, None, None, :] + wy[..., None, None] * rely[:, :, :, None, :, None]
            x = x + biases[0].reshape(b, t, nq, ch, 1, 1)
            for l in range(1, n_layers):
                x = F.relu(x)
                wl = weights[l].reshape(b * t * nq, ch, ch)
                x = torch.bmm(wl, x.reshape(b * t * nq, ch, h * w)).view(b, t, nq, ch, h, w) + biases[l].reshape(b, t, nq, ch, 1, 1)
            return x.reshape(b, t * nq, ch, h, w)


def build(args):
    if args.binary:
        num_classes = 1
    else:
        num_classes = {"ytvos": 65, "davis": 78, "a2d": 1, "jhmdb": 1}.get(args.dataset_file, 91)
    device = torch.device(args.device)
    if "video_swin" in args.backbone:
        from .video_swin_transformer import build_video_swin_backbone
        backbone = build_video_swin_backbone(args)
    elif "swin" in args.backbone:
        raise NotImplementedError("2-D Swin image backbones are out of scope (SURVEY.md section 2.1 #8)")
    else:
        backbone = build_backbone(args)
    transformer = build_deforamble_transformer(args)
    matcher = build_matcher(args)
    model = OCPG(args, backbone, transformer, num_classes=num_classes, num_queries=args.num_queries,
                 num_feature_levels=args.num_feature_levels, num_frames=args.num_frames, mask_dim=args.mask_dim,
                 dim_feedforward=args.dim_feedforward, controller_layers=args.controller_layers,
                 dynamic_mask_channels=args.dynamic_mask_channels, aux_loss=args.aux_loss,
                 with_box_refine=args.with_box_refine, two_stage=args.two_stage,
                 freeze_text_encoder=args.freeze_text_encoder, freeze_video_encoder=args.freeze_video_encoder,
                 rel_coord=args.rel_coord, matcher=matcher)
    weight_dict = {"loss_ce": args.cls_loss_coef, "loss_bbox": args.bbox_loss_coef, "loss_giou": args.giou_loss_coef}
    if args.masks:
        for suffix in ("", "_low"):
            weight_dict["loss_mask" + suffix] = args.mask_loss_coef
            weight_dict["loss_dice" + suffix] = args.dice_loss_coef
            weight_dict["loss_proj" + suffix] = args.proj_loss_coef
            weight_dict["loss_lst" + suffix] = args.lst_loss_coef
    if args.aux_loss:
        base = dict(weight_dict)
        for i in range(args.dec_layers - 1):
            weight_dict.update({f"{k}_{i}": v for k, v in base.items()})
    losses = ["labels", "boxes"] + (["masks"] if args.masks else [])
    criterion = SetCriterion(args, num_classes, matcher=matcher, weight_dict=weight_dict, eos_coef=args.eos_coef,
                             losses=losses, focal_alpha=args.focal_alpha)
    criterion.to(device)
    return model, criterion, build_postprocessors(args, args.dataset_file)
```

Measured before the change: 64.17.

## Pack all per-clip training targets in one fused native kernel shared by matcher and criterion

Adds a HIP kernel that builds every subsampled target map the matcher and criterion need in a single launch: gt masks at several strides, box region masks, weak masks, heat weights with a global min/max normalisation, and the resized region map. Previously these came from many small PyTorch ops (pad-stack, slicing, interpolate, box rasterisation), some of them run separately by the matcher and the criterion. The pack is built once per step and passed to both. The levelset loss also drops its zero-fill and atomic accumulation in favour of a deterministic two-kernel reduction. The cost is a large new code path whose results must match the PyTorch version, including NaN and box-edge handling.

```diff
diff --git a/include/ocpg_hip.h b/include/ocpg_hip.h
--- a/include/ocpg_hip.h
+++ b/include/ocpg_hip.h
@@ -334,6 +334,13 @@
                             const unsigned char* gt, const long long* gt_off, int max_out_h, int max_out_w, float thr, int invert,
                             int* counts, void* stream);
 
+long long ocpg_target_pack_workspace(int B);
+int ocpg_target_pack_f32(int B, int T, const void* const* masks, const void* const* heat, const void* const* weak, const int* hw,
+                         const void* const* boxes, const void* const* valid, const void* const* labels, const void* const* size, int PH,
+                         int PW, int s, int sl, int sm, int lh, int lw, float* gt_s, float* gt_m, float* region_s, float* region_l,
+                         float* region_ls, float* weak_s, float* weak_l, float* w_s, float* w_l, float* tboxes, float* valid_f,
+                         long long* valid_i, long long* labels_out, void* workspace, void* stream);
+
 const char* ocpg_hip_version(void);
 
 #ifdef __cplusplus
diff --git a/ocpg_amd/_lib.py b/ocpg_amd/_lib.py
--- a/ocpg_amd/_lib.py
+++ b/ocpg_amd/_lib.py
@@ -151,6 +151,8 @@
     "ocpg_refmask_counts_f32": [_vp] + [_int] * 5 + [_vp] * 4 + [_int, _int, ctypes.c_float, _int, _vp, _vp],
     "ocpg_sim_heat_workspace": [_int] * 4,
     "ocpg_sim_heat_f32": [_vp] + [_int] * 5 + [_vp] * 10,
+    "ocpg_target_pack_workspace": [_int],
+    "ocpg_target_pack_f32": [_int, _int] + [_vp] * 8 + [_int] * 7 + [_vp] * 15,
     "ocpg_win_attn_fwd": [_vp, _vp, _vp, ctypes.c_float] + [_int] * 5 + [_vp, _vp, _int, _vp],
     "ocpg_win_attn_bwd": [_vp, _vp, _vp, _vp, ctypes.c_float] + [_int] * 5 + [_vp] * 6 + [_int, _vp],
     "ocpg_win_attn_bwd_mfma": [_vp, _vp, _vp, _vp, ctypes.c_float] + [_int] * 5 + [_vp] * 6 + [_int, _vp],
@@ -254,6 +256,7 @@
         L.ocpg_groupnorm_cl_work.restype = ctypes.c_longlong
         L.ocpg_colsum_blocks.restype = ctypes.c_longlong
         L.ocpg_sim_heat_workspace.restype = ctypes.c_longlong
+        L.ocpg_target_pack_workspace.restype = ctypes.c_longlong
         _lib = _Lib(L)
     return _lib
 
diff --git a/ocpg_amd/csrc/levelset.hip b/ocpg_amd/csrc/levelset.hip
--- a/ocpg_amd/csrc/levelset.hip
+++ b/ocpg_amd/csrc/levelset.hip
@@ -2,7 +2,6 @@
 #include <stdint.h>
 
 #include "../../include/ocpg_hip.h"
-#include "fill.h"
 
 namespace {
 
@@ -86,12 +85,11 @@
   }
 }
 
-__global__ __launch_bounds__(64) void levelset_final(const float* __restrict__ part, int nblk, int N, int C, float* __restrict__ coef,
-                                                     float* __restrict__ loss) {
+__global__ __launch_bounds__(64) void levelset_final(float* __restrict__ part, int nblk, int N, int C, float* __restrict__ coef) {
   __shared__ float s[7 + 2 * CMAX];
   const int n = blockIdx.x, l = blockIdx.y;
   const int NS = 7 + 2 * C, NC = 8 + 2 * C;
-  const float* p = part + ((long long)l * N + n) * nblk * NS;
+  float* p = part + ((long long)l * N + n) * nblk * NS;
   for (int slot = 0; slot < NS; ++slot) {
     float v = 0.f;
     for (int b = threadIdx.x; b < nblk; b += 64) v += p[(long long)b * NS + slot];
@@ -123,7 +121,21 @@
   }
   k[6] = 1.f / ((float)C * pixels);
   k[7] = 0.00001f / pixels;
-  atomicAdd(loss + l, (e_tot / (float)C / pixels + 0.00001f * (s[4] + s[5]) / pixels) / (float)N);
+  p[0] = (e_tot / (float)C / pixels + 0.00001f * (s[4] + s[5]) / pixels) / (float)N;
+}
+
+__global__ __launch_bounds__(64) void levelset_total(const float* __restrict__ part, long long stride, int N, float* __restrict__ loss) {
+  __shared__ float t[64];
+  const float* p = part + (long long)blockIdx.x * N * stride;
+  float s = 0.f;
+  for (int n0 = 0; n0 < N; n0 += 64) {
+    __syncthreads();
+    if (n0 + (int)threadIdx.x < N) t[threadIdx.x] = p[(n0 + threadIdx.x) * stride];
+    __syncthreads();
+    if (threadIdx.x == 0)
+      for (int i = 0; i < 64 && n0 + i < N; ++i) s += t[i];
+  }
+  if (threadIdx.x == 0) loss[blockIdx.x] = s;
 }
 
 __global__ __launch_bounds__(256) void levelset_bwd(const float* __restrict__ x, const float* __restrict__ feats,
@@ -201,11 +213,10 @@
   hipStream_t st = (hipStream_t)stream;
   const int hw = h * w;
   const int nblk = (hw + 256 * PPT - 1) / (256 * PPT);
-  hipError_t e = ocpg_fill::zero_async(loss, sizeof(float) * (size_t)Lr, st);
-  if (e != hipSuccess) return -(int)e;
   levelset_sums<<<dim3(nblk, N, Lr), 256, 0, st>>>(x, feats, box, N, C, CF, h, w, sums);
-  levelset_final<<<dim3(N, Lr), 64, 0, st>>>(sums, nblk, N, C, coef, loss);
-  e = hipGetLastError();
+  levelset_final<<<dim3(N, Lr), 64, 0, st>>>(sums, nblk, N, C, coef);
+  levelset_total<<<Lr, 64, 0, st>>>(sums, (long long)nblk * (7 + 2 * C), N, loss);
+  const hipError_t e = hipGetLastError();
   return e == hipSuccess ? 0 : -(int)e;
 }
 
diff --git a/ocpg_amd/csrc/target_pack.hip b/ocpg_amd/csrc/target_pack.hip
--- /dev/null
+++ b/ocpg_amd/csrc/target_pack.hip
@@ -0,0 +1,277 @@
+#include <hip/hip_runtime.h>
+#include <stdint.h>
+
+#include "../../include/ocpg_hip.h"
+
+namespace {
+
+constexpr int NT = 256;
+constexpr int MAXB = 16;
+constexpr int NORM_BLOCKS = 1024;
+
+struct Clips {
+  const float* masks[MAXB];
+  const float* heat[MAXB];
+  const float* weak[MAXB];
+  const float* boxes[MAXB];
+  const long long* valid[MAXB];
+  const long long* labels[MAXB];
+  const long long* size[MAXB];
+  int H[MAXB], W[MAXB];
+};
+
+struct Outs {
+  float *gt_s, *gt_m, *region_s, *region_l, *region_ls, *weak_s, *weak_l, *w_s, *w_l, *tboxes, *valid_f;
+  long long *valid_i, *labels;
+};
+
+struct Geo {
+  int T, PH, PW, s, sl, sm, lh, lw;
+  int nb_s, nb_l, nb_m, nb_r;
+  int clip0;
+};
+
+struct Box {
+  int x0, x1, y0, y1;
+};
+
+__device__ __forceinline__ int slice_bound(int v, int size) { return v < 0 ? max(v + size, 0) : min(v, size); }
+
+__device__ __forceinline__ Box raster_box(const float* __restrict__ b, const long long* __restrict__ size, int PH, int PW) {
+  const float cx = b[0], cy = b[1], w = b[2], h = b[3];
+  const float fh = (float)size[0], fw = (float)size[1];
+  const int sx0 = (int)(fmaf(w, -0.5f, cx) * fw), sy0 = (int)(fmaf(h, -0.5f, cy) * fh);
+  const int sx1 = (int)(fmaf(w, 0.5f, cx) * fw), sy1 = (int)(fmaf(h, 0.5f, cy) * fh);
+  Box r = {0, 0, 0, 0};
+  if ((int)((unsigned)sy1 - (unsigned)sy0) > 0 && (int)((unsigned)sx1 - (unsigned)sx0) > 0) {
+    r.x0 = slice_bound(sx0, PW);
+    r.x1 = slice_bound(sx1, PW);
+    r.y0 = slice_bound(sy0, PH);
+    r.y1 = slice_bound(sy1, PH);
+  }
+  return r;
+}
+
+__device__ __forceinline__ float in_box(const Box& b, int y, int x) { return (y >= b.y0 && y < b.y1 && x >= b.x0 && x < b.x1) ? 1.f : 0.f; }
+
+__device__ __forceinline__ float fold_heat(float h) { return fabsf((h != h ? h : fminf(fmaxf(h, 0.3f), 0.7f)) - 0.5f); }
+
+__device__ __forceinline__ float nan_min(float a, float b) { return a != a ? a : (b != b ? b : fminf(a, b)); }
+__device__ __forceinline__ float nan_max(float a, float b) { return a != a ? a : (b != b ? b : fmaxf(a, b)); }
+
+__device__ __forceinline__ float4 read4(const float* __restrict__ src, int t, int H, int W, int y, int x0, int k) {
+  float4 v = make_float4(0.f, 0.f, 0.f, 0.f);
+  if (y >= H) return v;
+  const float* row = src + ((long long)t * H + y) * W;
+  if (k == 1 && x0 + 3 < W && (((uintptr_t)(row + x0)) & 15) == 0) return *reinterpret_cast<const float4*>(row + x0);
+  if (x0 < W) v.x = row[x0];
+  if (x0 + k < W) v.y = row[x0 + k];
+  if (x0 + 2 * k < W) v.z = row[x0 + 2 * k];
+  if (x0 + 3 * k < W) v.w = row[x0 + 3 * k];
+  return v;
+}
+
+__device__ __forceinline__ void store4(float* __restrict__ dst, long long off, float4 v) { *reinterpret_cast<float4*>(dst + off) = v; }
+
+__device__ __forceinline__ void block_minmax(float& lo, float& hi, float* red) {
+  for (int o = 32; o; o >>= 1) {
+    lo = nan_min(lo, __shfl_xor(lo, o));
+    hi = nan_max(hi, __shfl_xor(hi, o));
+  }
+  if ((threadIdx.x & 63) == 0) {
+    red[threadIdx.x >> 6] = lo;
+    red[NT / 64 + (threadIdx.x >> 6)] = hi;
+  }
+  __syncthreads();
+  lo = red[0];
+  hi = red[NT / 64];
+  for (int i = 1; i < NT / 64; ++i) {
+    lo = nan_min(lo, red[i]);
+    hi = nan_max(hi, red[NT / 64 + i]);
+  }
+}
+
+template <bool GT>
+__device__ __forceinline__ void pack_maps(const Clips& cl, int c, long long bc, const Geo& g, int k, int blk, int nblk, float* __restrict__ gt,
+                                          float* __restrict__ region, float* __restrict__ weak, float* __restrict__ wmap,
+                                          float* __restrict__ pmin, float* __restrict__ pmax, float* red) {
+  const int OH = g.PH / k, OW4 = g.PW / k / 4, H = cl.H[c], W = cl.W[c];
+  const long long nq = (long long)g.T * OH * OW4;
+  float lo = INFINITY, hi = -INFINITY;
+  for (long long q = (long long)blk * NT + threadIdx.x; q < nq; q += (long long)nblk * NT) {
+    const int ox = (int)(q % OW4) * 4;
+    const long long r = q / OW4;
+    const int oy = (int)(r % OH), t = (int)(r / OH);
+    const int y = oy * k + k / 2, x = ox * k + k / 2;
+    const Box b = raster_box(cl.boxes[c] + 4 * t, cl.size[c], g.PH, g.PW);
+    const float4 rg = make_float4(in_box(b, y, x), in_box(b, y, x + k), in_box(b, y, x + 2 * k), in_box(b, y, x + 3 * k));
+    const float4 wk = read4(cl.weak[c], t, H, W, y, x, k);
+    const float4 ht = read4(cl.heat[c], t, H, W, y, x, k);
+    const float4 a = make_float4(fold_heat(ht.x), fold_heat(ht.y), fold_heat(ht.z), fold_heat(ht.w));
+    lo = nan_min(nan_min(nan_min(lo, a.x), nan_min(a.y, a.z)), a.w);
+    hi = nan_max(nan_max(nan_max(hi, a.x), nan_max(a.y, a.z)), a.w);
+    const long long off = (((bc * g.T + t) * OH + oy) * OW4) * 4 + ox;
+    if (GT) store4(gt, off, read4(cl.masks[c], t, H, W, y, x, k));
+    store4(region, off, rg);
+    store4(weak, off, make_float4(wk.x * rg.x, wk.y * rg.y, wk.z * rg.z, wk.w * rg.w));
+    store4(wmap, off, a);
+  }
+  block_minmax(lo, hi, red);
+  if (threadIdx.x == 0) {
+    *pmin = lo;
+    *pmax = hi;
+  }
+}
+
+__global__ __launch_bounds__(NT) void tp_pack(const Clips cl, const Outs o, const Geo g, float* __restrict__ part, int np_s, int np_l) {
+  __shared__ float red[2 * NT / 64];
+  const int c = blockIdx.y;
+  const long long bc = g.clip0 + c;
+  int blk = blockIdx.x;
+  if (blk < g.nb_s) {
+    pack_maps<true>(cl, c, bc, g, g.s, blk, g.nb_s, o.gt_s, o.region_s, o.weak_s, o.w_s, part + bc * g.nb_s + blk,
+                    part + np_s + bc * g.nb_s + blk, red);
+    return;
+  }
+  blk -= g.nb_s;
+  if (blk < g.nb_l) {
+    pack_maps<false>(cl, c, bc, g, g.sl, blk, g.nb_l, nullptr, o.region_l, o.weak_l, o.w_l, part + 2ll * np_s + bc * g.nb_l + blk,
+                     part + 2ll * np_s + np_l + bc * g.nb_l + blk, red);
+    return;
+  }
+  blk -= g.nb_l;
+  if (blk < g.nb_m) {
+    const int k = g.sm, OH = g.PH / k, OW4 = g.PW / k / 4;
+    const long long nq = (long long)g.T * OH * OW4;
+    for (long long q = (long long)blk * NT + threadIdx.x; q < nq; q += (long long)g.nb_m * NT) {
+      const int ox = (int)(q % OW4) * 4;
+      const long long r = q / OW4;
+      const int oy = (int)(r % OH), t = (int)(r / OH);
+      store4(o.gt_m, (((bc * g.T + t) * OH + oy) * OW4) * 4 + ox, read4(cl.masks[c], t, cl.H[c], cl.W[c], oy * k + k / 2, ox * k + k / 2, k));
+    }
+    return;
+  }
+  blk -= g.nb_m;
+  if (blk < g.nb_r) {
+    const int k = g.s, IH = g.PH / k, IW = g.PW / k, OW4 = g.lw / 4;
+    const float sh = (float)IH / (float)g.lh, sw = (float)IW / (float)g.lw;
+    const long long nq = (long long)g.T * g.lh * OW4;
+    for (long long q = (long long)blk * NT + threadIdx.x; q < nq; q += (long long)g.nb_r * NT) {
+      const int ox = (int)(q % OW4) * 4;
+      const long long r = q / OW4;
+      const int oy = (int)(r % g.lh), t = (int)(r / g.lh);
+      const Box b = raster_box(cl.boxes[c] + 4 * t, cl.size[c], g.PH, g.PW);
+      const int y = min((int)floorf(oy * sh), IH - 1) * k + k / 2;
+      float v[4];
+#pragma unroll
+      for (int j = 0; j < 4; ++j) v[j] = in_box(b, y, min((int)floorf((ox + j) * sw), IW - 1) * k + k / 2);
+      store4(o.region_ls, (((bc * g.T + t) * g.lh + oy) * OW4) * 4 + ox, make_float4(v[0], v[1], v[2], v[3]));
+    }
+    return;
+  }
+  for (int t = threadIdx.x; t < g.T; t += NT) {
+    const long long i = bc * g.T + t;
+    const long long vd = cl.valid[c][t];
+    o.valid_i[i] = vd;
+    o.valid_f[i] = (float)vd;
+    if (o.labels) o.labels[i] = cl.labels[c][t];
+    store4(o.tboxes, 4 * i, make_float4(cl.boxes[c][4 * t], cl.boxes[c][4 * t + 1], cl.boxes[c][4 * t + 2], cl.boxes[c][4 * t + 3]));
+  }
+}
+
+__global__ __launch_bounds__(NT) void tp_normalise(float* __restrict__ w_s, const float* __restrict__ region_s, long long n4_s, int nbn_s,
+                                                   float* __restrict__ w_l, const float* __restrict__ region_l, long long n4_l,
+                                                   const float* __restrict__ part, int np_s, int np_l) {
+  __shared__ float red[2 * NT / 64];
+  const bool low = (int)blockIdx.x >= nbn_s;
+  const int blk = low ? blockIdx.x - nbn_s : blockIdx.x, nblk = low ? gridDim.x - nbn_s : nbn_s;
+  const float* pmin = low ? part + 2ll * np_s : part;
+  const int np = low ? np_l : np_s;
+  float lo = INFINITY, hi = -INFINITY;
+  for (int i = threadIdx.x; i < np; i += NT) {
+    lo = nan_min(lo, pmin[i]);
+    hi = nan_max(hi, pmin[np + i]);
+  }
+  block_minmax(lo, hi, red);
+  const float den = hi - lo + 1e-5f;
+  float4* w = reinterpret_cast<float4*>(low ? w_l : w_s);
+  const float4* rg = reinterpret_cast<const float4*>(low ? region_l : region_s);
+  const long long n4 = low ? n4_l : n4_s;
+  for (long long i = (long long)blk * NT + threadIdx.x; i < n4; i += (long long)nblk * NT) {
+    const float4 a = w[i], r = rg[i];
+    w[i] = make_float4(r.x == 0.f ? 1.f : (a.x - lo) / den, r.y == 0.f ? 1.f : (a.y - lo) / den, r.z == 0.f ? 1.f : (a.z - lo) / den,
+                       r.w == 0.f ? 1.f : (a.w - lo) / den);
+  }
+}
+
+inline int blocks_for(long long quads, int cap) {
+  const long long b = (quads + NT - 1) / NT;
+  return (int)(b < 1 ? 1 : (b > cap ? cap : b));
+}
+
+inline int clip_cap(int B) { return 1024 / B > 32 ? 1024 / B : 32; }
+
+inline bool misaligned(const void* p) { return ((uintptr_t)p & 15) != 0; }
+
+}
+
+extern "C" long long ocpg_target_pack_workspace(int B) { return B <= 0 ? 0 : 16ll * B * clip_cap(B); }
+
+extern "C" int ocpg_target_pack_f32(int B, int T, const void* const* masks, const void* const* heat, const void* const* weak, const int* hw,
+                                    const void* const* boxes, const void* const* valid, const void* const* labels, const void* const* size,
+                                    int PH, int PW, int s, int sl, int sm, int lh, int lw, float* gt_s, float* gt_m, float* region_s,
+                                    float* region_l, float* region_ls, float* weak_s, float* weak_l, float* w_s, float* w_l, float* tboxes,
+                                    float* valid_f, long long* valid_i, long long* labels_out, void* workspace, void* stream) {
+  if (B <= 0) return -1001;
+  if (T <= 0) return -1002;
+  if (!masks || !heat || !weak || !hw || !boxes || !valid || !size) return -1003;
+  if (PH <= 0 || PW <= 0) return -1005;
+  if (s <= 0 || sl <= 0 || sm <= 0) return -1006;
+  if (lh <= 0 || lw <= 0) return -1007;
+  for (int i = 0; i < B; ++i) {
+    if (!masks[i] || !heat[i] || !weak[i] || !boxes[i] || !valid[i] || !size[i] || (labels && !labels[i])) return -1003;
+    if (hw[2 * i] <= 0 || hw[2 * i] > PH || hw[2 * i + 1] <= 0 || hw[2 * i + 1] > PW) return -1004;
+  }
+  float* const maps[] = {gt_s, gt_m, region_s, region_l, region_ls, weak_s, weak_l, w_s, w_l, tboxes};
+  for (float* p : maps)
+    if (!p || misaligned(p)) return -1008;
+  if (!valid_f || !valid_i || (labels && !labels_out)) return -1009;
+  if (!workspace) return -1010;
+  for (int k : {s, sl, sm})
+    if (PH % k != 0 || PW % (4 * k) != 0) return -2000;
+  if (lw % 4 != 0) return -2000;
+  if ((long long)B * T * PH * PW >= (1ll << 40) || (long long)T * PH * PW >= (1ll << 31) || (long long)T * lh * lw >= (1ll << 31)) return -2000;
+
+  const int cap = clip_cap(B);
+  Geo g;
+  g.T = T, g.PH = PH, g.PW = PW, g.s = s, g.sl = sl, g.sm = sm, g.lh = lh, g.lw = lw;
+  g.nb_s = blocks_for((long long)T * (PH / s) * (PW / s / 4), cap);
+  g.nb_l = blocks_for((long long)T * (PH / sl) * (PW / sl / 4), cap);
+  g.nb_m = blocks_for((long long)T * (PH / sm) * (PW / sm / 4), cap);
+  g.nb_r = blocks_for((long long)T * lh * (lw / 4), cap);
+  const int np_s = B * g.nb_s, np_l = B * g.nb_l;
+  Outs o = {gt_s, gt_m, region_s, region_l, region_ls, weak_s, weak_l, w_s, w_l, tboxes, valid_f, valid_i, labels ? labels_out : nullptr};
+  hipStream_t st = (hipStream_t)stream;
+  for (int c0 = 0; c0 < B; c0 += MAXB) {
+    const int n = B - c0 < MAXB ? B - c0 : MAXB;
+    Clips cl = {};
+    for (int i = 0; i < n; ++i) {
+      cl.masks[i] = (const float*)masks[c0 + i];
+      cl.heat[i] = (const float*)heat[c0 + i];
+      cl.weak[i] = (const float*)weak[c0 + i];
+      cl.boxes[i] = (const float*)boxes[c0 + i];
+      cl.valid[i] = (const long long*)valid[c0 + i];
+      cl.labels[i] = labels ? (const long long*)labels[c0 + i] : nullptr;
+      cl.size[i] = (const long long*)size[c0 + i];
+      cl.H[i] = hw[2 * (c0 + i)];
+      cl.W[i] = hw[2 * (c0 + i) + 1];
+    }
+    g.clip0 = c0;
+    tp_pack<<<dim3((unsigned)(g.nb_s + g.nb_l + g.nb_m + g.nb_r + 1), (unsigned)n), NT, 0, st>>>(cl, o, g, (float*)workspace, np_s, np_l);
+  }
+  const long long n4_s = (long long)B * T * (PH / s) * (PW / s / 4), n4_l = (long long)B * T * (PH / sl) * (PW / sl / 4);
+  const int nbn_s = blocks_for(n4_s, NORM_BLOCKS), nbn_l = blocks_for(n4_l, NORM_BLOCKS);
+  tp_normalise<<<(unsigned)(nbn_s + nbn_l), NT, 0, st>>>(w_s, region_s, n4_s, nbn_s, w_l, region_l, n4_l, (const float*)workspace, np_s, np_l);
+  const hipError_t e = hipGetLastError();
+  return e == hipSuccess ? 0 : -(int)e;
+}
diff --git a/ocpg_amd/models/criterion.py b/ocpg_amd/models/criterion.py
--- a/ocpg_amd/models/criterion.py
+++ b/ocpg_amd/models/criterion.py
@@ -3,21 +3,14 @@
 from torch import nn
 
 from ..util import box_ops
-from ..util.misc import get_world_size, is_dist_avail_and_initialized, nested_tensor_from_tensor_list
+from ..util.misc import get_world_size, is_dist_avail_and_initialized
 from .matcher import _assert_well_formed, _pairwise_giou_1
 from .ops.functions import mask_loss_func
-from .segmentation import generate_box_region_mask
+from .ops.functions.target_pack_func import build_target_pack
 
 HIP_MASK_LOSSES = True
 HIP_DET_LOSSES = True
-
-
-def _pad_stack(targets, key):
-    return nested_tensor_from_tensor_list([t[key] for t in targets], size_divisibility=32, split=False).decompose()[0]
-
-
-def _sub(x, k):
-    return x[..., k // 2::k, k // 2::k]
+MASK_OUT_STRIDE, MASK_OUT_STRIDE_LOW = 1, 2
 
 
 def _dice(x, t):
@@ -39,8 +32,8 @@
         empty_weight[-1] = self.eos_coef
         self.register_buffer("empty_weight", empty_weight)
         self.focal_alpha = focal_alpha
-        self.mask_out_stride = 1
-        self.mask_out_stride_low = 2
+        self.mask_out_stride = MASK_OUT_STRIDE
+        self.mask_out_stride_low = MASK_OUT_STRIDE_LOW
         self.iter = 0
         self._warmup_iters = 100000
         self.iter_device = None
@@ -75,31 +68,24 @@
         giou = (1 - _pairwise_giou_1(sx, tx)).sum((1, 2)) / num_boxes
         return l1, giou
 
-    def _masks_stacked(self, pm, pml, src_lst, targets, num_boxes, warm):
+    def _pack(self, targets, ls_hw, pack=None):
+        s, sl = self.mask_out_stride, self.mask_out_stride_low
+        ls_hw = (int(ls_hw[0]), int(ls_hw[1]))
+        if pack is not None and pack.targets is targets and pack.key[:2] == (s, sl) and pack.key[3] == ls_hw:
+            return pack
+        return build_target_pack(targets, s, sl, self.matcher.mask_out_stride if self.matcher is not None else 2, ls_hw)
+
+    def _masks_stacked(self, pm, pml, src_lst, targets, num_boxes, warm, pack=None):
         with torch.autocast(device_type=pm.device.type, enabled=False):
-            return self._masks_stacked_fp32(pm.float(), pml.float(), src_lst.float(), targets, num_boxes, warm)
-
-    def _masks_stacked_fp32(self, pm, pml, src_lst, targets, num_boxes, warm):
+            return self._masks_stacked_fp32(pm.float(), pml.float(), src_lst.float(), targets, num_boxes, warm, pack)
+
+    def _masks_stacked_fp32(self, pm, pml, src_lst, targets, num_boxes, warm, pack=None):
         lr = pm.shape[0]
-        gt = _pad_stack(targets, "masks").to(pml)
-        heat = _pad_stack(targets, "weights").to(pml)
-        weak = _pad_stack(targets, "weak_masks").to(pml)
-        s, sl = self.mask_out_stride, self.mask_out_stride_low
-        im_h, im_w = gt.shape[-2:]
-        b, nf = weak.shape[:2]
-        gt_full = _sub(gt, s)
-        assert gt_full.size(2) * s == im_h and gt_full.size(3) * s == im_w
-        sizes = torch.stack([t["size"] for t in targets]).repeat_interleave(nf, dim=0)
-        boxes = box_ops.box_cxcywh_to_xyxy(torch.cat([t["boxes"] for t in targets], dim=0))
-        region = generate_box_region_mask(boxes, (im_h, im_w), sizes).view(b, nf, im_h, im_w)
-        region_low, region = _sub(region, sl), _sub(region, s)
-        weak_full, weak_low = _sub(weak, s) * region, _sub(weak, sl) * region_low
-
-        def heat_weight(h, reg):
-            w = (h.clamp(min=0.3, max=0.7) - 0.5).abs()
-            lo, hi = w.min(), w.max()
-            w = (w - lo) / (hi - lo + 1e-5)
-            return torch.where(reg == 0, torch.ones_like(w), w)
+        lst_hw = src_lst.shape[-2:]
+        pack = self._pack(targets, lst_hw, pack)
+        gt_full, region, region_low, region_scaled = pack.gt_s, pack.region_s, pack.region_l, pack.region_ls
+        weak_full, weak_low, w_full, w_low = pack.weak_s, pack.weak_l, pack.w_s, pack.w_l
+        b, nf = weak_full.shape[:2]
 
         def masked_ce(x, w, m):
             return F.binary_cross_entropy_with_logits(x.sigmoid() * w, (m * w).expand_as(x), reduction="none").mean((1, 2, 3, 4))
@@ -128,14 +114,11 @@
                 return (v[..., 1:, :] - v[..., :-1, :]).abs().sum((2, 3)) + (v[..., :, 1:] - v[..., :, :-1]).abs().sum((2, 3))
             return (region_e / pixels + 0.00001 * (length(fg) + length(bg)) / pixels).mean(1)
 
-        w_full, w_low = heat_weight(_sub(heat, s), region), heat_weight(_sub(heat, sl), region_low)
         if pm.is_cuda and HIP_MASK_LOSSES and pm[0].numel() % 4 == 0 and pml[0].numel() % 4 == 0:
             loss_mask, loss_mask_low = mask_loss_func.masked_ce(pm, w_full, weak_full), mask_loss_func.masked_ce(pml, w_low, weak_low)
         else:
             loss_mask, loss_mask_low = masked_ce(pm, w_full, weak_full), masked_ce(pml, w_low, weak_low)
-        lst_hw = src_lst.shape[-2:]
         scaled = F.interpolate(pm.flatten(0, 1), lst_hw, mode="bilinear", align_corners=True).view(lr, b * nf, *lst_hw)
-        region_scaled = F.interpolate(region, lst_hw, mode="nearest").flatten(0, 1)
         feats = src_lst.flatten(0, 1)[:, :-1]
         if pm.is_cuda and HIP_MASK_LOSSES and feats.shape[1] <= 16:
             full_feats = src_lst.flatten(0, 1)
@@ -211,16 +194,24 @@
 
         losses, maps = {}, (None, None, None)
         per_layer = {}
+        pack = outputs.get("_target_pack")
+        if pack is not None and pack.targets is not targets:
+            pack = None
+        if "masks" in self.losses:
+            pack = self._pack(targets, outputs["ls_features"].shape[-2:], pack)
         if HIP_DET_LOSSES and "labels" in self.losses and "boxes" in self.losses and src.is_cuda:
             from .matcher import _BOX_ERRORS
             dev = src.device
             flag = _BOX_ERRORS.get(dev)
             if flag is None and not torch.cuda.is_current_stream_capturing():
                 flag = _BOX_ERRORS[dev] = torch.zeros((), dtype=torch.int32, device=dev)
-            valid = torch.stack([t["valid"] for t in targets]).to(dev)
-            labels = None if self.num_classes == 1 else torch.stack([t["labels"] for t in targets]).to(dev)
-            tboxes = torch.stack([t["boxes"] for t in targets]).to(dev)
-            det = mask_loss_func.det_losses(stacked("pred_logits"), stacked("pred_boxes"), src, valid, labels, tboxes, num_boxes,
+            if pack is not None:
+                valid, labels, tboxes = pack.valid_f, None if self.num_classes == 1 else pack.labels, pack.tboxes
+            else:
+                valid = torch.stack([t["valid"] for t in targets]).to(dev)
+                labels = None if self.num_classes == 1 else torch.stack([t["labels"] for t in targets]).to(dev)
+                tboxes = torch.stack([t["boxes"] for t in targets]).to(dev)
+            det =mask_loss_func.det_losses(stacked("pred_logits"), stacked("pred_boxes"), src, valid, labels, tboxes, num_boxes,
                                             self.focal_alpha, flag)
             per_layer["loss_ce"], per_layer["loss_bbox"], per_layer["loss_giou"] = det.unbind(0)
         else:
@@ -230,7 +221,7 @@
                 per_layer["loss_bbox"], per_layer["loss_giou"] = self._boxes_stacked(stacked("pred_boxes"), src, targets, num_boxes)
         if "masks" in self.losses:
             warm = self._warm(len(layers)).to(outputs["pred_masks_low"].device)
-            d, maps = self._masks_stacked(stacked("pred_masks"), stacked("pred_masks_low"), outputs["ls_features"], targets, num_boxes, warm)
+            d, maps = self._masks_stacked(stacked("pred_masks"), stacked("pred_masks_low"), outputs["ls_features"], targets, num_boxes, warm, pack)
             per_layer.update(d)
         order = [k for k in ("loss_ce", "loss_bbox", "loss_giou", "loss_proj", "loss_mask", "loss_lst", "loss_proj_low", "loss_mask_low",
                              "loss_lst_low") if k in per_layer]
diff --git a/ocpg_amd/models/matcher.py b/ocpg_amd/models/matcher.py
--- a/ocpg_amd/models/matcher.py
+++ b/ocpg_amd/models/matcher.py
@@ -3,7 +3,7 @@
 from torch import nn
 
 from ..util.box_ops import box_cxcywh_to_xyxy
-from ..util.misc import nested_tensor_from_tensor_list
+from .ops.functions.target_pack_func import matcher_targets
 
 
 def _pairwise_giou_1(boxes, tgt):
@@ -54,20 +54,18 @@
         self.mask_out_stride = 2
 
     @torch.no_grad()
-    def cost_matrix_stacked(self, logits, boxes, masks, targets):
+    def cost_matrix_stacked(self, logits, boxes, masks, targets, pack=None):
         with torch.autocast(device_type=masks.device.type, enabled=False):
             logits, boxes, masks = logits.float(), boxes.float(), masks.float()
             lr, bs, nf, nq, h, w = masks.shape
-            gt, _ = nested_tensor_from_tensor_list([t["masks"] for t in targets], size_divisibility=32, split=False).decompose()
-            gt = gt.to(masks)
             s = self.mask_out_stride
-            im_h, im_w = gt.shape[-2:]
-            gt = gt[:, :, s // 2::s, s // 2::s]
-            assert gt.size(2) * s == im_h and gt.size(3) * s == im_w
-
-            valid = torch.stack([t["valid"] for t in targets]).to(logits.dtype)
+            if pack is not None and pack.targets is targets and pack.key[2] == s:
+                gt, valid, tb, labels = pack.gt_m, pack.valid_f, pack.tboxes, pack.labels
+            else:
+                gt, valid, tb, labels = matcher_targets(targets, s, labels=self.num_classes != 1)
+                gt, valid, tb = gt.to(masks), valid.to(logits.dtype), tb.to(boxes.dtype)
             if masks.is_cuda and HIP_MATCHER:
-                return self._cost_matrix_hip(logits, boxes, masks, gt, valid, targets)
+                return self._cost_matrix_hip(logits, boxes, masks, gt, valid, tb, None if self.num_classes == 1 else labels)
             prob = logits.sigmoid()
             alpha, gamma = 0.25, 2.0
             neg = (1 - alpha) * (prob ** gamma) * (-(1 - prob + 1e-8).log())
@@ -75,11 +73,10 @@
             if self.num_classes == 1:
                 cls = (pos - neg)[..., 0]
             else:
-                ids = torch.stack([t["labels"] for t in targets])
+                ids = labels
                 cls = torch.gather(pos - neg, 4, ids[None, :, :, None, None].expand(lr, -1, -1, nq, 1))[..., 0]
             cost_class = (cls * valid[None, :, :, None]).sum(2) / valid.sum(1)[None, :, None]
 
-            tb = torch.stack([t["boxes"] for t in targets]).to(boxes.dtype)
             cost_bbox = (boxes - tb[None, :, :, None, :]).abs().sum(-1).mean(2)
             pb, tbx = box_cxcywh_to_xyxy(boxes), box_cxcywh_to_xyxy(tb)
             _assert_well_formed(pb, "predictions")
@@ -97,14 +94,14 @@
             return (self.cost_class * cost_class + self.cost_bbox * cost_bbox + self.cost_giou * cost_giou
                     + self.cost_mask * cost_mask + self.cost_dice * cost_dice)
 
-    def _cost_matrix_hip(self, logits, boxes, masks, gt, valid, targets):
+    def _cost_matrix_hip(self, logits, boxes, masks, gt, valid, tb, labels):
         from .._lib import check, lib
         lr, bs, nf, nq, h, w = masks.shape
         if masks.stride(-1) != 1 or masks.stride(-2) != w:
             masks = masks.contiguous()
         logits, boxes, gt = logits.contiguous(), boxes.contiguous(), gt.contiguous()
-        tb = torch.stack([t["boxes"] for t in targets]).to(boxes.dtype).contiguous()
-        labels = None if self.num_classes == 1 else torch.stack([t["labels"] for t in targets]).to(torch.int64).contiguous()
+        tb = tb.contiguous()
+        labels = None if labels is None else labels.contiguous()
         flag = _BOX_ERRORS.get(masks.device)
         if flag is None and not torch.cuda.is_current_stream_capturing():
             flag = _BOX_ERRORS[masks.device] = torch.zeros((), dtype=torch.int32, device=masks.device)
@@ -124,8 +121,8 @@
         return self.cost_matrix_stacked(outputs["pred_logits"][None], outputs["pred_boxes"][None], outputs["pred_masks"][None], targets)[0]
 
     @torch.no_grad()
-    def match_stacked(self, logits, boxes, masks, targets):
-        return self.cost_matrix_stacked(logits, boxes, masks, targets).argmin(dim=2)
+    def match_stacked(self, logits, boxes, masks, targets, pack=None):
+        return self.cost_matrix_stacked(logits, boxes, masks, targets, pack).argmin(dim=2)
 
     @staticmethod
     def as_indices(src):
diff --git a/ocpg_amd/models/ocpg.py b/ocpg_amd/models/ocpg.py
--- a/ocpg_amd/models/ocpg.py
+++ b/ocpg_amd/models/ocpg.py
@@ -10,7 +10,8 @@
 from ..util.misc import NestedTensor, inverse_sigmoid, nested_tensor_from_videos_list, resize_mask
 from . import amp_cache
 from .backbone import build_backbone
-from .criterion import SetCriterion
+from .criterion import MASK_OUT_STRIDE, MASK_OUT_STRIDE_LOW, SetCriterion
+from .ops.functions.target_pack_func import CRITERION_KEYS, build_target_pack
 from .decoder import MSO
 from .deformable_transformer import build_deforamble_transformer
 from .matcher import build_matcher
@@ -320,8 +321,12 @@
         if self.training:
             shuffled = sh_all.permute(2, 0, 1, 3, 4, 5)
             with torch.no_grad():
+                pack = None
+                if self.aux_loss and all(k in targets[0] for k in CRITERION_KEYS):
+                    pack = out["_target_pack"] = build_target_pack(targets, MASK_OUT_STRIDE, MASK_OUT_STRIDE_LOW, self.matcher.mask_out_stride,
+                                                                   (4 * tar[0], 4 * tar[1]))
                 if self.aux_loss:
-                    src_all = self.matcher.match_stacked(outputs_class, outputs_coord, shuffled, targets)
+                    src_all = self.matcher.match_stacked(outputs_class, outputs_coord, shuffled, targets, pack)
                 else:
                     src_all = self.matcher.match_stacked(outputs_class[-1:], outputs_coord[-1:], shuffled[-1:], targets)
                 out["pred_masks"] = seg_masks_shuffled[-1]
diff --git a/ocpg_amd/models/ops/functions/target_pack_func.py b/ocpg_amd/models/ops/functions/target_pack_func.py
--- /dev/null
+++ b/ocpg_amd/models/ops/functions/target_pack_func.py
@@ -0,0 +1,129 @@
+import ctypes
+import os
+from types import SimpleNamespace
+
+import torch
+import torch.nn.functional as F
+
+from ....util import box_ops
+from ....util.misc import nested_tensor_from_tensor_list
+
+NATIVE = os.environ.get("OCPG_TARGET_PACK", "1") != "0"
+
+CRITERION_KEYS = ("masks", "weights", "weak_masks", "boxes", "valid", "size")
+
+
+def _pad_stack(targets, key):
+    return nested_tensor_from_tensor_list([t[key] for t in targets], size_divisibility=32, split=False).decompose()[0]
+
+
+def _sub(x, k):
+    return x[..., k // 2::k, k // 2::k]
+
+
+def heat_weight(h, reg):
+    w = (h.clamp(min=0.3, max=0.7) - 0.5).abs()
+    lo, hi = w.min(), w.max()
+    w = (w - lo) / (hi - lo + 1e-5)
+    return torch.where(reg == 0, torch.ones_like(w), w)
+
+
+def matcher_targets(targets, sm, labels=True):
+    gt, _ = nested_tensor_from_tensor_list([t["masks"] for t in targets], size_divisibility=32, split=False).decompose()
+    gt = gt.to(torch.float32)
+    im_h, im_w = gt.shape[-2:]
+    gt = gt[:, :, sm // 2::sm, sm // 2::sm]
+    assert gt.size(2) * sm == im_h and gt.size(3) * sm == im_w
+    valid = torch.stack([t["valid"] for t in targets]).to(torch.float32)
+    tb = torch.stack([t["boxes"] for t in targets]).to(torch.float32)
+    lab = torch.stack([t["labels"] for t in targets]).to(torch.int64) if labels and "labels" in targets[0] else None
+    return gt, valid, tb, lab
+
+
+def _compose(targets, s, sl, sm, ls_hw):
+    from ...segmentation import generate_box_region_mask
+    gt = _pad_stack(targets, "masks").to(torch.float32)
+    heat = _pad_stack(targets, "weights").to(torch.float32)
+    weak = _pad_stack(targets, "weak_masks").to(torch.float32)
+    im_h, im_w = gt.shape[-2:]
+    b, nf = weak.shape[:2]
+    gt_full = _sub(gt, s)
+    assert gt_full.size(2) * s == im_h and gt_full.size(3) * s == im_w
+    sizes = torch.stack([t["size"] for t in targets]).repeat_interleave(nf, dim=0)
+    boxes = box_ops.box_cxcywh_to_xyxy(torch.cat([t["boxes"] for t in targets], dim=0))
+    region = generate_box_region_mask(boxes, (im_h, im_w), sizes).view(b, nf, im_h, im_w)
+    region_low, region = _sub(region, sl), _sub(region, s)
+    weak_full, weak_low = _sub(weak, s) * region, _sub(weak, sl) * region_low
+    w_full, w_low = heat_weight(_sub(heat, s), region), heat_weight(_sub(heat, sl), region_low)
+    region_scaled = F.interpolate(region, tuple(ls_hw), mode="nearest").flatten(0, 1)
+    gt_m, valid_f, tboxes, labels = matcher_targets(targets, sm)
+    return SimpleNamespace(gt_s=gt_full, gt_m=gt_m, region_s=region, region_l=region_low, region_ls=region_scaled, weak_s=weak_full,
+                           weak_l=weak_low, w_s=w_full, w_l=w_low, tboxes=tboxes, valid_f=valid_f,
+                           valid_i=torch.stack([t["valid"] for t in targets]), labels=labels)
+
+
+def _ceil32(v):
+    return (v + 31) // 32 * 32
+
+
+def _native(targets, s, sl, sm, ls_hw):
+    from ...._lib import check, lib
+    b = len(targets)
+    dev = targets[0]["masks"].device
+    keep = []
+
+    def ptrs(key, dtype):
+        ts = [t[key].to(dtype).contiguous() for t in targets]
+        keep.append(ts)
+        return (ctypes.c_void_p * b)(*[x.data_ptr() for x in ts]), ts
+
+    masks, m = ptrs("masks", torch.float32)
+    heat, h = ptrs("weights", torch.float32)
+    weak, w = ptrs("weak_masks", torch.float32)
+    nf = m[0].shape[0]
+    for i in range(b):
+        assert m[i].ndim == 3 and m[i].shape == h[i].shape == w[i].shape and m[i].shape[0] == nf, "masks / weights / weak_masks disagree"
+        assert targets[i]["boxes"].shape == (nf, 4) and targets[i]["valid"].shape == (nf,) and targets[i]["size"].shape == (2,)
+    boxes, _ = ptrs("boxes", torch.float32)
+    valid, _ = ptrs("valid", torch.int64)
+    size, _ = ptrs("size", torch.int64)
+    labels = None
+    if "labels" in targets[0]:
+        labels, lab = ptrs("labels", torch.int64)
+        assert all(x.shape == (nf,) for x in lab)
+    hw = (ctypes.c_int * (2 * b))(*[v for x in m for v in x.shape[1:]])
+    ph, pw = _ceil32(max(x.shape[1] for x in m)), _ceil32(max(x.shape[2] for x in m))
+    lh, lw = int(ls_hw[0]), int(ls_hw[1])
+
+    def f32(*shape):
+        return torch.empty(shape, dtype=torch.float32, device=dev)
+
+    p = SimpleNamespace(gt_s=f32(b, nf, ph // s, pw // s), gt_m=f32(b, nf, ph // sm, pw // sm), region_s=f32(b, nf, ph // s, pw // s),
+                        region_l=f32(b, nf, ph // sl, pw // sl), region_ls=f32(b * nf, lh, lw), weak_s=f32(b, nf, ph // s, pw // s),
+                        weak_l=f32(b, nf, ph // sl, pw // sl), w_s=f32(b, nf, ph // s, pw // s), w_l=f32(b, nf, ph // sl, pw // sl),
+                        tboxes=f32(b, nf, 4), valid_f=f32(b, nf), valid_i=torch.empty((b, nf), dtype=torch.int64, device=dev),
+                        labels=None if labels is None else torch.empty((b, nf), dtype=torch.int64, device=dev))
+    ws = torch.empty((max(int(lib().ocpg_target_pack_workspace(b)), 16),), dtype=torch.uint8, device=dev)
+    rc = lib().ocpg_target_pack_f32(b, nf, masks, heat, weak, hw, boxes, valid, labels, size, ph, pw, s, sl, sm, lh, lw, p.gt_s.data_ptr(),
+                                    p.gt_m.data_ptr(), p.region_s.data_ptr(), p.region_l.data_ptr(), p.region_ls.data_ptr(),
+                                    p.weak_s.data_ptr(), p.weak_l.data_ptr(), p.w_s.data_ptr(), p.w_l.data_ptr(), p.tboxes.data_ptr(),
+                                    p.valid_f.data_ptr(), p.valid_i.data_ptr(), None if p.labels is None else p.labels.data_ptr(),
+                                    ws.data_ptr(), torch.cuda.current_stream().cuda_stream)
+    if rc == -2000:
+        return None
+    check(rc, "ocpg_target_pack_f32")
+    return p
+
+
+def build_target_pack(targets, s, sl, sm, ls_hw, native=None):
+    if native is None:
+        native = NATIVE
+    ls_hw = (int(ls_hw[0]), int(ls_hw[1]))
+    p = None
+    if native and targets[0]["masks"].is_cuda:
+        p = _native(targets, s, sl, sm, ls_hw)
+    if p is None:
+        with torch.no_grad(), torch.autocast(device_type=targets[0]["masks"].device.type, enabled=False):
+            p = _compose(targets, s, sl, sm, ls_hw)
+    p.targets, p.key = targets, (s, sl, sm, ls_hw)
+    return p
```

New measurement: 65.02 (median of 6 runs). +1.3%, better.
